# nmonette/TO-UED

Measured on NVIDIA B200. Metric: gridworld agent env-steps/sec incl. LPG update, higher is better.
Workload: dtype f16/bf16 operands, f32 accumulate (GRU); f32 elsewhere

## Files before the change

include/toued.h:

```cpp
#ifndef TOUED_H
#define TOUED_H
#include <stdint.h>
#ifdef __cplusplus
extern "C" {
#endif

#define TOUED_LEVEL_BYTES 192

const char* toued_last_error(void);
int toued_version(void);

int toued_rollout(const void* levels, const uint32_t* keys, const float* actor,
                  const uint8_t* forced_actions, int32_t* state, int32_t* obs, uint8_t* action,
                  float* reward, uint8_t* done, float* ep_return, int n_agents, int n_workers,
                  int rollout_len, int obs_dim, int max_grid_size, int max_n_objs, int reset_first,
                  void* stream);

int toued_env_step(const void* levels, const uint32_t* keys, const int32_t* actions, int32_t* state,
                   int32_t* obs, float* reward, uint8_t* done, int n_agents, int n_workers,
                   int max_grid_size, int max_n_objs, void* stream);
int toued_env_reset(const void* levels, int32_t* state, int32_t* obs, int n_agents, int n_workers,
                    int max_grid_size, void* stream);


int toued_sort_tokens(const int32_t* obs, uint16_t* sorted_tok, int n_agents, int n_workers,
                      int rollout_len, void* stream);

int toued_lpg_prepare(const int32_t* obs, const uint8_t* action, const float* reward,
                      const uint8_t* done, const float* actor, const float* critic,
                      const float* lpg_params, const int32_t* step, const void* levels, float* x,
                      void* ximg, int n_agents, int n_workers, int rollout_len, int obs_dim,
                      int lifetime_conditioning, int lpg_stride, void* stream);

int toued_gru_forward(const float* x, const uint8_t* done, const float* lpg_params, float* h_out,
                      float* gates, float* pi_hat, float* y_hat, int n_agents, int n_workers,
                      int rollout_len, int lifetime_conditioning, int lpg_stride, void* stream);

int toued_agent_scratch_floats(int n_agents, int n_workers, int rollout_len, int obs_dim);
int toued_agent_update(const int32_t* obs, const uint8_t* action, const uint16_t* sorted_tok,
                       const float* pi_hat, const float* y_hat, const float* actor_in,
                       const float* critic_in, float* actor_out, float* critic_out,
                       const void* levels, int32_t* step, float* scalars, int n_agents,
                       int n_workers, int rollout_len, int obs_dim, float lr_actor, float lr_critic,
                       float max_grad_norm, float agent_target_coeff, int tables_precopied, float* run_scratch,
                       void* stream);


int toued_meta_loss(const int32_t* obs, const uint8_t* action, const float* reward,
                    const uint8_t* done, const uint16_t* sorted_tok, const float* value_table,
                    const float* actor, float* lam, float* mu, float* scalars, int n_agents,
                    int n_workers, int rollout_len, int obs_dim, int value_stride, float gamma,
                    float gae_lambda, float grad_scale, int outer_product_quirk, void* stream);

int toued_agent_backward(const int32_t* obs, const uint8_t* action, const uint16_t* sorted_tok,
                         const float* pi_hat, const float* y_hat, const float* actor_k,
                         const float* critic_k, const float* actor_k1, const float* critic_k1,
                         const float* update_scalars, float* lam, float* mu, float* d_pi_hat,
                         float* d_y_hat, int n_agents, int n_workers, int rollout_len, int obs_dim,
                         float lr_actor, float lr_critic, float max_grad_norm,
                         float agent_target_coeff, float policy_entropy_coeff,
                         float target_entropy_coeff, float policy_l2_coeff, float target_l2_coeff,
                         float grad_scale, float* run_scratch, void* stream);

int toued_transpose_wh(const float* lpg_params, float* whT, void* stream);

int toued_gru_backward(const uint8_t* done, const float* lpg_params, const float* whT,
                       const float* h, float* gates, const float* y_hat, const float* d_pi_hat,
                       const float* d_y_hat, float* dl, float* dx, int n_agents, int n_workers,
                       int rollout_len, int lifetime_conditioning, void* stream);

int toued_lpg_wgrad_workspace_floats(void);
int toued_lpg_wgrad(const int32_t* obs, const uint8_t* done, const float* critic,
                    const float* lpg_params, const float* x, const float* h, const float* dgates,
                    const float* d_pi_hat, const float* dl, const float* dx, float* workspace,
                    int n_agents, int n_workers, int rollout_len, int obs_dim,
                    int lifetime_conditioning, int accumulate, void* stream);
int toued_lpg_wgrad_workspace_offset(int which);
int toued_lpg_wgrad_embed(const int32_t* obs, const uint8_t* done, const float* critic, const float* lpg_params,
                          const float* dx, float* workspace, const uint32_t* cotangent_max, int n_agents, int n_workers,
                          int rollout_len, int obs_dim, int lifetime_conditioning, int accumulate, void* stream);
int toued_lpg_wgrad_splits(int which);
int toued_reduce_partials(const float* workspace, float* grad, int lifetime_conditioning, int wh_splits,
                          int sm_splits, void* stream);

int toued_adam(float* params, const float* grad, float* mu, float* nu, int n, int count, float lr,
               float b1, float b2, float eps, void* stream);
int toued_adam_dev(float* params, const float* grad, float* mu, float* nu, int* count_dev, int n, float lr,
                   float b1, float b2, float eps, void* stream);
int toued_sgd_clip(float* params, const float* grad, float* sqnorm_scratch, int n, float lr, float max_norm,
                   void* stream);

int toued_a2c_update(const int32_t* obs, const uint8_t* action, const float* reward, const uint8_t* done,
                     const uint16_t* sorted_tok, const float* actor_in, const float* critic_in,
                     float* actor_out, float* critic_out, const void* levels, int32_t* step,
                     float* scalars, int n_agents, int n_workers, int rollout_len, int obs_dim,
                     float lr_actor, float lr_critic, float max_grad_norm, float gamma, float gae_lambda,
                     float entropy_coeff, int outer_product_quirk, void* stream);

int toued_a2c_train(const void* levels, const uint32_t* keys, float* actor0, float* actor1, float* critic0,
                    float* critic1, int32_t* state, int32_t* obs, uint8_t* action, float* reward, uint8_t* done,
                    uint16_t* sorted_tok, int32_t* step, float* scalars, float* loss_sums, int num_updates,
                    int n_agents, int n_workers, int rollout_len, int obs_dim, int max_grid_size, int max_n_objs,
                    float lr_actor, float lr_critic, float max_grad_norm, float gamma, float gae_lambda,
                    float entropy_coeff, int outer_product_quirk, void* stream);

int toued_es_ask(const uint32_t* key, const float* mean, float sigma, float* candidates, int popsize,
                 int n_params, int cand_stride, void* stream);
int toued_es_tell(const float* candidates, const float* fitness, float* mean, float* m, float* v,
                  int popsize, int n_params, int cand_stride, float sigma, float lrate, float beta1,
                  float beta2, float eps, int gen_counter, float mean_decay, void* stream);

int toued_es_ask_shard(const uint32_t* key, const float* mean, float sigma, float* candidates, int popsize_global,
                       int n_params, int cand_stride, int pair_offset, int n_pairs, void* stream);
int toued_es_grad_partial(const float* candidates, const float* fitness, const float* mean, float* grad_sum,
                          int n_members, int n_params, int cand_stride, float sigma, void* stream);
int toued_es_adam(const float* grad_sum, float* mean, float* m, float* v, int popsize_global, int n_params,
                  float sigma, float lrate, float beta1, float beta2, float eps, int gen_counter, float mean_decay,
                  void* stream);

int toued_plr_reset_lowest(float* score, uint8_t* active, uint8_t* is_new, int buffer_size, int minimum_new,
                           int* reset_ids, void* stream);
int toued_plr_select(uint32_t key0, uint32_t key1, float* score, uint8_t* active, uint8_t* is_new, int buffer_size,
                     const int* old_ids, const uint8_t* terminated, const float* new_scores, int n_agents,
                     float p_replay, float temperature, int shuffle_rounds, int* new_ids, void* stream);

int toued_generate_levels_desc_bytes(void);
int toued_generate_levels(const void* gen_desc, const uint32_t* keys, const int32_t* buffer_ids, void* levels_out,
                          int32_t* lifetimes_out, int n_levels, void* stream);

int toued_get_nash(const float* game, const float* x0, const float* y0, float* x_out, float* y_out,
                   int n, int x_nz, int y_nz, int num_iters, float lr, void* stream);
int toued_projection_simplex(float* v, int n, int max_nz, void* stream);


int toued_init_tables(const uint32_t* keys, const uint8_t* mask, float* tables, int n_agents,
                      int obs_dim, int n_out, void* stream);
int toued_masked_reset(const void* levels, const uint8_t* mask, int32_t* state, int32_t* obs,
                       int32_t* step, int n_agents, int n_workers, int max_grid_size, void* stream);

int toued_host_iota_bits(const uint32_t* keys, int n_keys, int n, uint32_t* out);


int toued_key_split(const uint32_t* keys_in, int n_keys, int num, int offset, int count, uint32_t* out,
                    void* stream);
int toued_key_chain(const uint32_t* keys_in, int n_keys, int chain_len, uint32_t* keys_out,
                    uint32_t* carry_out, void* stream);


int toued_tc_gemm_test(const float* A, const float* B, void* scratch_img, float* D, void* stream);
int toued_tc_gemm_mixed_test(const float* A, const float* B, void* scratch_img, float* D, void* stream);
int toued_tc_gemm_mn_test(const float* A, const float* B, void* scratch_img, float* D, int lbo, int sbo,
                          int kadv, void* stream);
int toued_tc_gemm_mn2_test(const float* A, const float* B, void* scratch_img, float* D, void* stream);

int toued_pack_wh_forward(const float* lpg_params, void* wh_img, int lifetime_conditioning, void* stream);
int toued_gru_forward_tc(const float* x, const uint8_t* done, const float* lpg_params, const void* wh_img,
                         void* h16, void* fac, void* hpimg, float* pi_hat, float* y_hat, int n_agents,
                         int n_workers, int rollout_len, int lifetime_conditioning, void* stream);
int toued_pack_wh_forward_multi(const float* lpg_params, void* wh_img, int lifetime_conditioning, int n_sets,
                                int lpg_stride, void* stream);
int toued_gru_forward_tc_multi(const float* x, const uint8_t* done, const float* lpg_params, const void* wh_img,
                               float* pi_hat, float* y_hat, int n_agents, int n_workers, int rollout_len,
                               int lifetime_conditioning, int lpg_stride, void* stream);

int toued_pack_wh_backward(const float* lpg_params, void* whb_img, void* stream);
int toued_cotangent_max(const float* d_pi_hat, const float* d_y_hat, int n_agents, int n_workers, int rollout_len,
                        uint32_t* cotangent_max, void* stream);
int toued_gru_backward_tc(const uint8_t* done, const float* lpg_params, const void* whb_img,
                          const void* h16, const void* fac, const float* y_hat, const float* d_pi_hat,
                          const float* d_y_hat, void* dgimg, float* dl, float* dx, const uint32_t* cotangent_max,
                          int n_agents, int n_workers, int rollout_len, int lifetime_conditioning, void* stream);
int toued_wgrad_tc_splits(void);
int toued_wgrad_tc_small_splits(void);
int toued_lpg_wgrad_tc(const void* hpimg, const void* dgimg, const void* ximg, const void* h16,
                       const float* d_pi_hat, const float* dl, float* wh_partials, float* small_partials,
                       const uint32_t* cotangent_max, int n_agents, int n_workers, int rollout_len, int accumulate,
                       void* stream);

#ifdef __cplusplus
}
#endif
#endif
```

to_ued_b200/_lib.py:

```python
from __future__ import annotations

import ctypes as C
import os

_HERE = os.path.dirname(os.path.abspath(__file__))
_VARIANT = os.environ.get("TOUED_LIB_VARIANT", "")
LIB_PATH = os.path.join(_HERE, f"libtoued_{_VARIANT}.so" if _VARIANT else "libtoued.so")

_lib = None


class TouedError(RuntimeError):
    pass


def lib() -> C.CDLL:
    global _lib
    if _lib is None:
        if not os.path.exists(LIB_PATH):
            raise TouedError(
                f"{LIB_PATH} is missing: the CUDA extension is not built. "
                "Run `python -m to_ued_b200.csrc.build` (there is no CPU fallback).")
        _lib = C.CDLL(LIB_PATH)
        _declare(_lib)
    return _lib


_P, _I, _F = C.c_void_p, C.c_int, C.c_float

SIGNATURES = {
    "toued_rollout": [_P] * 10 + [_I] * 7 + [_P],
    "toued_env_step": [_P] * 7 + [_I] * 4 + [_P],
    "toued_env_reset": [_P] * 3 + [_I] * 3 + [_P],
    "toued_sort_tokens": [_P] * 2 + [_I] * 3 + [_P],
    "toued_lpg_prepare": [_P] * 11 + [_I] * 6 + [_P],
    "toued_gru_forward": [_P] * 7 + [_I] * 5 + [_P],
    "toued_agent_update": [_P] * 12 + [_I] * 4 + [_F] * 4 + [_I, _P, _P],
    "toued_agent_scratch_floats": [_I] * 4,
    "toued_meta_loss": [_P] * 10 + [_I] * 5 + [_F] * 3 + [_I, _P],
    "toued_agent_backward": [_P] * 14 + [_I] * 4 + [_F] * 9 + [_P, _P],
    "toued_transpose_wh": [_P] * 3,
    "toued_gru_backward": [_P] * 10 + [_I] * 4 + [_P],
    "toued_lpg_wgrad_workspace_floats": [],
    "toued_lpg_wgrad": [_P] * 11 + [_I] * 6 + [_P],
    "toued_reduce_partials": [_P, _P, _I, _I, _I, _P],
    "toued_lpg_wgrad_splits": [_I],
    "toued_lpg_wgrad_workspace_offset": [_I],
    "toued_lpg_wgrad_embed": [_P] * 7 + [_I] * 6 + [_P],
    "toued_cotangent_max": [_P, _P, _I, _I, _I, _P, _P],
    "toued_pack_wh_backward": [_P] * 3,
    "toued_gru_backward_tc": [_P] * 12 + [_I] * 4 + [_P],
    "toued_wgrad_tc_splits": [],
    "toued_wgrad_tc_small_splits": [],
    "toued_lpg_wgrad_tc": [_P] * 9 + [_I] * 4 + [_P],
    "toued_adam": [_P] * 4 + [_I, _I] + [_F] * 4 + [_P],
    "toued_adam_dev": [_P] * 5 + [_I] + [_F] * 4 + [_P],
    "toued_sgd_clip": [_P] * 3 + [_I, _F, _F, _P],
    "toued_get_nash": [_P] * 5 + [_I] * 4 + [_F, _P],
    "toued_projection_simplex": [_P, _I, _I, _P],
    "toued_es_ask": [_P, _P, _F, _P, _I, _I, _I, _P],
    "toued_es_tell": [_P] * 5 + [_I, _I, _I] + [_F] * 5 + [_I, _F, _P],
    "toued_es_ask_shard": [_P, _P, _F, _P, _I, _I, _I, _I, _I, _P],
    "toued_es_grad_partial": [_P] * 4 + [_I, _I, _I, _F, _P],
    "toued_es_adam": [_P] * 4 + [_I, _I] + [_F] * 5 + [_I, _F, _P],
    "toued_a2c_update": [_P] * 12 + [_I] * 4 + [_F] * 6 + [_I, _P],
    "toued_a2c_train": [_P] * 15 + [_I] * 7 + [_F] * 6 + [_I, _P],
    "toued_init_tables": [_P] * 3 + [_I] * 3 + [_P],
    "toued_masked_reset": [_P] * 5 + [_I] * 3 + [_P],
    "toued_generate_levels_desc_bytes": [],
    "toued_generate_levels": [_P] * 5 + [_I, _P],
    "toued_plr_reset_lowest": [_P] * 3 + [_I, _I, _P, _P],
    "toued_plr_select": [C.c_uint32, C.c_uint32] + [_P] * 3 + [_I] + [_P] * 3 + [_I, _F, _F, _I, _P, _P],
    "toued_tc_gemm_test": [_P] * 5,
    "toued_tc_gemm_mixed_test": [_P] * 5,
    "toued_tc_gemm_mn_test": [_P] * 4 + [_I] * 3 + [_P],
    "toued_tc_gemm_mn2_test": [_P] * 5,
    "toued_pack_wh_forward": [_P, _P, _I, _P],
    "toued_pack_wh_forward_multi": [_P, _P, _I, _I, _I, _P],
    "toued_gru_forward_tc_multi": [_P] * 6 + [_I] * 5 + [_P],
    "toued_host_iota_bits": [_P, _I, _I, _P],
    "toued_key_split": [_P, _I, _I, _I, _I, _P, _P],
    "toued_key_chain": [_P, _I, _I, _P, _P, _P],
    "toued_gru_forward_tc": [_P] * 9 + [_I] * 4 + [_P],
}


def _declare(l):
    l.toued_last_error.restype = C.c_char_p
    l.toued_last_error.argtypes = []
    l.toued_version.restype = _I
    l.toued_version.argtypes = []
    for name, args in SIGNATURES.items():
        fn = getattr(l, name)
        fn.restype = _I
        fn.argtypes = args


def ptr(t):
    if t is None:
        return None
    if not t.is_cuda:
        raise TouedError("to_ued_b200 ops need CUDA tensors (there is no CPU fallback)")
    if not t.is_contiguous():
        raise TouedError("to_ued_b200 ops need contiguous tensors")
    return t.data_ptr()


def stream_ptr():
    import torch
    return torch.cuda.current_stream().cuda_stream


KERNELS_PER_CALL = {"toued_adam_dev": 2, "toued_sgd_clip": 2, "toued_lpg_wgrad": 3, "toued_init_tables": 2, "toued_lpg_wgrad_tc": 2, "toued_pack_wh_forward": 2, "toued_pack_wh_forward_multi": 2}
LAUNCHES = {}
GRAPH_KERNELS = [0]
ENV_STEPS = [0]
PROFILE = None


H2D_BYTES = [0]


def h2d(t):
    H2D_BYTES[0] += int(t.numel() * t.element_size()) if hasattr(t, "element_size") else int(t.nbytes)
    return t


def reset_counters(profile=False):
    global PROFILE
    H2D_BYTES[0] = 0
    GRAPH_KERNELS[0] = 0
    ENV_STEPS[0] = 0
    LAUNCHES.clear()
    PROFILE = {} if profile else None


def kernel_launches():
    return sum(n * KERNELS_PER_CALL.get(k, 1) for k, n in LAUNCHES.items()) + GRAPH_KERNELS[0]


def profile_ms():
    return {k: (len(v), sum(a.elapsed_time(b) for a, b in v)) for k, v in (PROFILE or {}).items()}


def call(name, *args):
    LAUNCHES[name] = LAUNCHES.get(name, 0) + 1
    if name == "toued_rollout":
        ENV_STEPS[0] += args[10] * args[11] * args[12]
    elif name == "toued_a2c_train":
        ENV_STEPS[0] += args[15] * args[16] * args[17] * args[18]
    if PROFILE is not None:
        import torch
        a, b = torch.cuda.Event(enable_timing=True), torch.cuda.Event(enable_timing=True)
        a.record()
        rc = getattr(lib(), name)(*args)
        b.record()
        PROFILE.setdefault(name, []).append((a, b))
    else:
        rc = getattr(lib(), name)(*args)
    if rc != 0:
        raise TouedError(f"{name} failed ({rc}): {lib().toued_last_error().decode()}")
```

to_ued_b200/agents/lpg_agent.py:

```python
from __future__ import annotations

from dataclasses import dataclass, field
from typing import Any, List, Optional

import numpy as np
import torch

from .. import _lib
from ..util import prng
from ..util.data import AgentState, Transition


@dataclass
class LPGAgentMetrics:
    policy_l2: Any
    policy_entropy: Any
    critic_loss: Any
    critic_l2: Any
    critic_entropy: Any

    def as_dict(self):
        return {"policy_l2": self.policy_l2, "policy_entropy": self.policy_entropy,
                "critic_loss": self.critic_loss, "critic_l2": self.critic_l2,
                "critic_entropy": self.critic_entropy}


class Tape:

    def __init__(self, n_agents, n_workers, rollout_len, obs_dim, num_updates, device, keep_gates=True,
                 precision=None, per_agent_params=False):
        import to_ued_b200
        N, W, L, D, K = n_agents, n_workers, rollout_len, obs_dim, num_updates
        R, dev = N * W, device
        f32, u8, i32 = torch.float32, torch.uint8, torch.int32
        self.N, self.W, self.L, self.D, self.K, self.R = N, W, L, D, K, R
        self.record = bool(keep_gates)
        kt = K + 1 if self.record else 2
        kr = K + 1 if self.record else 1
        ka = K if self.record else 1
        self.kt, self.kr, self.ka = kt, kr, ka
        self.actor = torch.empty((kt, N, D, 8), dtype=f32, device=dev)
        self.critic = torch.empty((kt, N, D, 8), dtype=f32, device=dev)
        self.obs = torch.empty((kr, N, L + 1, W), dtype=i32, device=dev)
        self.action = torch.empty((kr, N, L, W), dtype=u8, device=dev)
        self.reward = torch.empty((kr, N, L, W), dtype=f32, device=dev)
        self.done = torch.empty((kr, N, L, W), dtype=u8, device=dev)
        self.sorted_tok = torch.empty((kr, N, L * W), dtype=torch.int16, device=dev)
        self.precision = precision or to_ued_b200.GRU_PRECISION
        self.x = torch.empty((ka, L, R, 8), dtype=f32, device=dev)
        self.ximg = None
        if self.precision == "tc":
            f16 = torch.float16
            Rp = (R + 63) // 64 * 64
            R32 = (R + 31) // 32 * 32
            self.h16 = None if per_agent_params else torch.empty((ka, L, R32, 256), dtype=f16, device=dev)
            self.fac = torch.empty((ka, 4, L, R32, 256), dtype=f16, device=dev) if self.record else None
            self.hpimg = torch.zeros((ka, L * Rp * 256 * 2), dtype=torch.uint8, device=dev) if self.record else None
            self.ximg = torch.zeros((ka, L * Rp * 128), dtype=torch.uint8, device=dev) if self.record else None
            self.wh_img = torch.zeros((N if per_agent_params else 1) * 16 * 26624 // 2, dtype=f16, device=dev)
            self.h = self.gates = None
        else:
            self.h = torch.empty((ka, L, R, 256), dtype=f32, device=dev)
            self.gates = torch.empty((ka, 4, L, R, 256), dtype=f32, device=dev) if self.record else None
        self.pi_hat = torch.empty((ka, L, R), dtype=f32, device=dev)
        self.y_hat = torch.empty((ka, L, R, 8), dtype=f32, device=dev)
        self.scalars = torch.empty((ka, N, 8), dtype=f32, device=dev)
        self.scal_sum = torch.zeros((N, 8), dtype=f32, device=dev)
        self.step_in = torch.empty((ka, N), dtype=i32, device=dev)
        self.ep_return = torch.empty((N, W), dtype=f32, device=dev)
        self.agent_scratch = torch.empty(_lib.lib().toued_agent_scratch_floats(N, W, L, D), dtype=f32, device=dev)

    def ti(self, k):
        return k if self.record else (k & 1)

    def ri(self, k):
        return k if self.record else 0

    def ai(self, k):
        return k if self.record else 0

    def transition(self, k) -> Transition:
        r = self.ri(k)
        return Transition(self.obs[r], self.action[r], self.reward[r], self.done[r])


_SORT_STREAMS = {}


def _sort_stream(cur):
    key = (cur.device.index, cur.cuda_stream)
    st = _SORT_STREAMS.get(key)
    if st is None:
        st = _SORT_STREAMS[key] = torch.cuda.Stream(device=cur.device)
    return st


def _mark(label):
    import to_ued_b200
    if to_ued_b200.PHASE_EVENTS is not None and getattr(to_ued_b200, "PHASE_FINE", False):
        e = torch.cuda.Event(enable_timing=True)
        e.record(torch.cuda.current_stream())
        to_ued_b200.PHASE_EVENTS.append((label, -2, e))


def lpg_agent_train_step(k, tape: Tape, levels, step, lpg_params, lifetime_conditioning, agent_target_coeff,
                         lr_actor, lr_critic, max_grad_norm, lpg_stride=0):
    N, W, L, D = tape.N, tape.W, tape.L, tape.D
    s = _lib.stream_ptr()
    p = _lib.ptr
    r, a, t0, t1 = tape.ri(k), tape.ai(k), tape.ti(k), tape.ti(k + 1)
    import to_ued_b200
    cur = torch.cuda.current_stream()
    side = _sort_stream(cur) if to_ued_b200.SIDE_STREAMS else cur
    ev_roll, ev_sort = torch.cuda.Event(), torch.cuda.Event()
    ev_roll.record(cur)
    with torch.cuda.stream(side):
        side.wait_event(ev_roll)
        _lib.call("toued_sort_tokens", p(tape.obs[r]), p(tape.sorted_tok[r]), N, W, L, _lib.stream_ptr())
        precopied = bool(to_ued_b200.SIDE_STREAMS)
        if precopied:
            tape.actor[t1].copy_(tape.actor[t0])
            tape.critic[t1].copy_(tape.critic[t0])
        ev_sort.record(side)
    _mark("rollout")
    tape.step_in[a].copy_(step)
    _lib.call("toued_lpg_prepare", p(tape.obs[r]), p(tape.action[r]), p(tape.reward[r]), p(tape.done[r]),
              p(tape.actor[t0]), p(tape.critic[t0]), p(lpg_params), p(step), p(levels), p(tape.x[a]),
              p(tape.ximg[a]) if tape.ximg is not None else None,
              N, W, L, D, int(lifetime_conditioning), int(lpg_stride), s)
    if lpg_stride and tape.precision == "tc":
        _lib.call("toued_gru_forward_tc_multi", p(tape.x[a]), p(tape.done[r]), p(lpg_params), p(tape.wh_img),
                  p(tape.pi_hat[a]), p(tape.y_hat[a]), N, W, L, int(lifetime_conditioning), int(lpg_stride), s)
    elif lpg_stride or tape.precision != "tc":
        _lib.call("toued_gru_forward", p(tape.x[a]), p(tape.done[r]), p(lpg_params), p(tape.h[a]),
                  p(tape.gates[a]) if tape.gates is not None else None, p(tape.pi_hat[a]), p(tape.y_hat[a]),
                  N, W, L, int(lifetime_conditioning), int(lpg_stride), s)
    else:
        _lib.call("toued_gru_forward_tc", p(tape.x[a]), p(tape.done[r]), p(lpg_params), p(tape.wh_img),
                  p(tape.h16[a]), p(tape.fac[a]) if tape.fac is not None else None,
                  p(tape.hpimg[a]) if tape.hpimg is not None else None, p(tape.pi_hat[a]), p(tape.y_hat[a]),
                  N, W, L, int(lifetime_conditioning), s)
    _mark("gru_fwd")
    cur.wait_event(ev_sort)
    _mark("sort_wait")
    _lib.call("toued_agent_update", p(tape.obs[r]), p(tape.action[r]), p(tape.sorted_tok[r]), p(tape.pi_hat[a]),
              p(tape.y_hat[a]), p(tape.actor[t0]), p(tape.critic[t0]), p(tape.actor[t1]), p(tape.critic[t1]),
              p(levels), p(step), p(tape.scalars[a]), N, W, L, D, float(lr_actor), float(lr_critic),
              float(max_grad_norm), float(agent_target_coeff), int(precopied), p(tape.agent_scratch), s)
    tape.scal_sum += tape.scalars[a]
    _mark("update")


def train_lpg_agent_steps(rng, lpg_train_state, agent_state: AgentState, rollout_manager, num_train_steps: int,
                          agent_target_coeff: float, tape: Optional[Tape] = None, lpg_stride: int = 0):
    env = rollout_manager.env
    actor, critic = agent_state.actor_state, agent_state.critic_state
    N, W = agent_state.env_state.packed.shape
    L, K = rollout_manager.train_rollout_len, num_train_steps
    dev = actor.params.device
    if tape is None:
        import to_ued_b200
        tape = Tape(N, W, L, env.obs_dim, K, dev, keep_gates=False,
                    precision=to_ued_b200.ES_PRECISION if lpg_stride else None, per_agent_params=bool(lpg_stride))
    levels = agent_state.level.packed
    step = actor.step.clone()
    state = agent_state.env_state.packed.clone()
    tape.actor[0].copy_(actor.params)
    tape.critic[0].copy_(critic.params)
    tape.scal_sum.zero_()
    keys_d = prng.chain_device(prng.to_device(rng, dev), K)
    p = _lib.ptr
    lpg = lpg_train_state.params if hasattr(lpg_train_state, "params") else lpg_train_state
    cond = lpg_train_state.model.lifetime_conditioning if hasattr(lpg_train_state, "model") else False
    if tape.precision == "tc" and not lpg_stride:
        _lib.call("toued_pack_wh_forward", p(lpg), p(tape.wh_img), int(cond), _lib.stream_ptr())
    elif tape.precision == "tc":
        _lib.call("toued_pack_wh_forward_multi", p(lpg), p(tape.wh_img), int(cond), N, int(lpg_stride), _lib.stream_ptr())
    yield
    for k in range(K):
        r = tape.ri(k)
        _lib.call("toued_rollout", p(levels), p(keys_d[k]), p(tape.actor[tape.ti(k)]), None, p(state), p(tape.obs[r]),
                  p(tape.action[r]), p(tape.reward[r]), p(tape.done[r]), None, N, W, L, env.obs_dim,
                  env.max_grid_size, env.max_n_objs, 0, _lib.stream_ptr())
        lpg_agent_train_step(k, tape, levels, step, lpg, cond, agent_target_coeff, actor.learning_rate,
                             critic.learning_rate, actor.max_grad_norm, lpg_stride=lpg_stride)
        yield
    sc = tape.scal_sum / K
    metrics = LPGAgentMetrics(policy_l2=sc[:, 4], policy_entropy=sc[:, 6], critic_loss=sc[:, 3],
                              critic_l2=sc[:, 5], critic_entropy=sc[:, 7])
    from ..environments.gridworld.gridworld import EnvState
    new_agent = agent_state.replace(
        actor_state=actor.replace(params=tape.actor[tape.ti(K)].clone(), step=step),
        critic_state=critic.replace(params=tape.critic[tape.ti(K)].clone(), step=step.clone()),
        env_obs=tape.obs[tape.ri(K - 1)][:, -1].clone(), env_state=EnvState(state, env.max_n_objs))
    rollouts = [tape.transition(k) for k in range(K)] if tape.record else [tape.transition(K - 1)]
    return new_agent, rollouts, metrics


def train_lpg_agent(rng, lpg_train_state, agent_state: AgentState, rollout_manager, num_train_steps: int,
                    agent_target_coeff: float, tape: Optional[Tape] = None, lpg_stride: int = 0):
    gen = train_lpg_agent_steps(rng, lpg_train_state, agent_state, rollout_manager, num_train_steps,
                                agent_target_coeff, tape=tape, lpg_stride=lpg_stride)
    while True:
        try:
            next(gen)
        except StopIteration as done:
            return done.value
```

to_ued_b200/csrc/agent_backward.cu:

```cuda
#include "lpg_common.cuh"
#include "segreduce.cuh"
#include "../../include/toued.h"

__global__ void __launch_bounds__(256)
meta_loss_kernel(const int32_t* __restrict__ obs, const uint8_t* __restrict__ action,
                 const float* __restrict__ reward, const uint8_t* __restrict__ done,
                 const uint16_t* __restrict__ sorted_tok, const float* __restrict__ value,
                 const float* __restrict__ actor, float* __restrict__ lam, float* __restrict__ mu,
                 float* __restrict__ scal, int W, int L, int D, int vstride, float gamma, float lmbda,
                 float gscale, int quirk) {
    extern __shared__ __align__(16) float sm[];
    float* adv = sm;
    float* rec = adv + L * W;
    float* abar = rec + L * W * 6;
    float* lbar = abar + W;
    float* runv = lbar + W;
    float* scan = runv + L * W * 5;
    void* idxmem = scan + 2 * 256 * 5;
    __shared__ float red[32];
    __shared__ int iscan[512];
    __shared__ unsigned char sflags[512];
    const int n = blockIdx.x, tid = threadIdx.x, T = W * L;
    const int32_t* ob = obs + (size_t)n * (L + 1) * W;
    const uint8_t* act = action + (size_t)n * T;
    const float* rw = reward + (size_t)n * T;
    const uint8_t* dn = done + (size_t)n * T;
    const uint16_t* st = sorted_tok + (size_t)n * T;
    const float* vt = value + (size_t)n * D * vstride;
    const float* at = actor + (size_t)n * D * 8;
    float* lm = lam + (size_t)n * D * 8;
    float* mm = mu + (size_t)n * D * 8;
    const float invT = 1.0f / (float)T;
    const SegIndex si = seg_index_build(idxmem, iscan, st, ob, T);

    for (int i = tid; i < D * 2; i += 256) {
        reinterpret_cast<float4*>(lm)[i] = make_float4(0.f, 0.f, 0.f, 0.f);
        reinterpret_cast<float4*>(mm)[i] = make_float4(0.f, 0.f, 0.f, 0.f);
    }
    float s1 = 0.f, s2 = 0.f;
    const float vlast = vt[(size_t)(D - 1) * vstride];
    for (int w = tid; w < W; w += 256) {
        float g = 0.f;
        int32_t o1 = ob[L * W + w];
        float v1 = vt[(size_t)ob_idx(o1) * vstride] + 0.001f * (float)ob_time(o1) * vlast;
        for (int t = L - 1; t >= 0; --t) {
            const int32_t o0 = ob[t * W + w];
            const float v0 = vt[(size_t)ob_idx(o0) * vstride] + 0.001f * (float)ob_time(o0) * vlast;
            const float nd = dn[t * W + w] ? 0.0f : 1.0f;
            const float delta = rw[t * W + w] + gamma * v1 * nd - v0;
            g = delta + gamma * lmbda * nd * g;
            adv[t * W + w] = g;
            s1 += g; s2 = fmaf(g, g, s2);
            v1 = v0;
        }
    }
    s1 = block_sum(s1, red); s2 = block_sum(s2, red);
    const float mean = s1 * invT;
    float var = 0.f;
    for (int i = tid; i < T; i += 256) { const float d = adv[i] - mean; var = fmaf(d, d, var); }
    var = block_sum(var, red) * invT;
    const float inv_std = 1.0f / (sqrtf(var) + 1e-8f);
    __syncthreads();
    for (int i = tid; i < T; i += 256) adv[i] = (adv[i] - mean) * inv_std;
    __syncthreads();
    for (int tok = tid; tok < T; tok += 256) {
        const int32_t o = ob[tok];
        float z[5], p[5];
        tab_logits8<5>(at, D, o, z);
        softmax_c<5>(z, p);
        const int a = act[tok];
        float pa = p[0];
#pragma unroll
        for (int j = 1; j < 5; ++j) pa = (a == j) ? p[j] : pa;
        float* r = rec + tok * 6;
        r[5] = logf(pa + 1e-8f);
        const float q = pa / (pa + 1e-8f);
#pragma unroll
        for (int j = 0; j < 5; ++j) r[j] = q * ((a == j ? 1.0f : 0.0f) - p[j]);
    }
    __syncthreads();
    float loss = 0.f;
    for (int w = tid; w < W; w += 256) {
        float sa = 0.f, sl = 0.f, se = 0.f;
        for (int t = 0; t < L; ++t) { sa += adv[t * W + w]; sl += rec[(t * W + w) * 6 + 5]; se = fmaf(adv[t * W + w], rec[(t * W + w) * 6 + 5], se); }
        abar[w] = sa / (float)L; lbar[w] = sl / (float)L;
        loss -= quirk ? abar[w] * lbar[w] : se / (float)L;
    }
    loss = block_sum(loss, red) / (float)W;
    __syncthreads();
    float last[5] = {0.f, 0.f, 0.f, 0.f, 0.f};
    for (int tok = tid; tok < T; tok += 256) {
        const int w = tok % W;
        const float coef = -gscale * invT * (quirk ? abar[w] : adv[tok]);
        float* r = rec + tok * 6;
        const float tf = 0.001f * (float)ob_time(ob[tok]);
#pragma unroll
        for (int j = 0; j < 5; ++j) { r[j] *= coef; last[j] = fmaf(tf, r[j], last[j]); }
        r[5] = tf;
    }
#pragma unroll
    for (int j = 0; j < 5; ++j) last[j] = block_sum(last[j], red);
    __syncthreads();
    seg_reduce<5, 6>(rec, si, T, runv, scan, sflags);
    for (int r = tid; r < si.nruns; r += 256) {
        const int row = si.run_row[r];
#pragma unroll
        for (int j = 0; j < 5; ++j) lm[(size_t)row * 8 + j] = runv[r * 5 + j];
    }
    if (tid == 0) {
#pragma unroll
        for (int j = 0; j < 5; ++j) lm[(size_t)(D - 1) * 8 + j] = last[j];
        scal[n * 2 + 0] = loss;
        scal[n * 2 + 1] = s2 * invT;
    }
}

extern "C" int toued_meta_loss(const int32_t* obs, const uint8_t* action, const float* reward,
                               const uint8_t* done, const uint16_t* sorted_tok, const float* value_table,
                               const float* actor, float* lam, float* mu, float* scalars, int n_agents,
                               int n_workers, int rollout_len, int obs_dim, int value_stride, float gamma,
                               float gae_lambda, float grad_scale, int outer_product_quirk, void* stream) {
    const int T = n_workers * rollout_len;
    TOUED_CHECK(n_agents > 0 && T > 0, "toued_meta_loss: empty problem");
    const size_t smem = sizeof(float) * ((size_t)T * 7 + 2 * n_workers + (size_t)T * 5 + 2 * 256 * 5) + seg_index_bytes(T);
    TOUED_CHECK(smem <= 200 * 1024, "toued_meta_loss: W*L=%d too large for shared memory", T);
    TOUED_CUDA(cudaFuncSetAttribute(meta_loss_kernel, cudaFuncAttributeMaxDynamicSharedMemorySize, (int)smem));
    meta_loss_kernel<<<n_agents, 256, smem, (cudaStream_t)stream>>>(
        obs, action, reward, done, sorted_tok, value_table, actor, lam, mu, scalars, n_workers, rollout_len,
        obs_dim, value_stride, gamma, gae_lambda, grad_scale, outer_product_quirk);
    TOUED_LAUNCH_CHECK();
    return 0;
}

struct TokFwd { float p[5], y[8], pa, q, tf; int a; };

__device__ __forceinline__ TokFwd tok_forward(const float* at, const float* ct, int D, int32_t o, int a) {
    TokFwd f;
    float z[5], zy[8];
    tab_logits8<5>(at, D, o, z);
    softmax_c<5>(z, f.p);
    tab_logits8<8>(ct, D, o, zy);
    softmax_c<8>(zy, f.y);
    f.a = a;
    f.pa = f.p[0];
#pragma unroll
    for (int j = 1; j < 5; ++j) f.pa = (a == j) ? f.p[j] : f.pa;
    f.q = f.pa / (f.pa + 1e-8f);
    f.tf = 0.001f * (float)ob_time(o);
    return f;
}

__device__ __forceinline__ void tok_grad(const TokFwd& f, float ph, const float* yh, float invT, float alpha, float* c) {
    const float ca = invT * ph * f.q;
#pragma unroll
    for (int j = 0; j < 5; ++j) c[j] = ca * ((f.a == j ? 1.0f : 0.0f) - f.p[j]);
    float mm[8], b = 0.f;
#pragma unroll
    for (int i = 0; i < 8; ++i) {
        mm[i] = logf(f.y[i] + 1e-8f) - logf(yh[i] + 1e-8f) + f.y[i] / (f.y[i] + 1e-8f);
        b = fmaf(f.y[i], mm[i], b);
    }
    const float cc = alpha * invT;
#pragma unroll
    for (int i = 0; i < 8; ++i) c[5 + i] = cc * f.y[i] * (mm[i] - b);
}

__device__ __forceinline__ void load8(const float* p, float* v) {
    const float4 a = reinterpret_cast<const float4*>(p)[0], b = reinterpret_cast<const float4*>(p)[1];
    v[0] = a.x; v[1] = a.y; v[2] = a.z; v[3] = a.w; v[4] = b.x; v[5] = b.y; v[6] = b.z; v[7] = b.w;
}

__global__ void __launch_bounds__(256, 2)
agent_backward_kernel(const int32_t* __restrict__ obs, const uint8_t* __restrict__ action,
                      const uint16_t* __restrict__ sorted_tok, const float* __restrict__ pi_hat,
                      const float* __restrict__ y_hat, const float* __restrict__ actor_k,
                      const float* __restrict__ critic_k, const float* __restrict__ actor_k1,
                      const float* __restrict__ critic_k1, const float* __restrict__ upd_scal,
                      float* lam, float* mu, float* __restrict__ d_pi_hat, float* __restrict__ d_y_hat,
                      float* run_scratch, int n_agents, int W, int L, int D, float lr_a, float lr_c, float max_norm,
                      float alpha, float b_pent, float b_yent, float b_pl2, float b_yl2, float gscale) {
    extern __shared__ __align__(16) float rec[];
    __shared__ float red[32];
    __shared__ float s_wlast[13];
    __shared__ int iscan[512];
    __shared__ unsigned char sflags[512];
    const int n = blockIdx.x, tid = threadIdx.x, T = W * L, R = n_agents * W;
    const int32_t* ob = obs + (size_t)n * (L + 1) * W;
    const uint8_t* act = action + (size_t)n * T;
    const uint16_t* st = sorted_tok + (size_t)n * T;
    const float* a0 = actor_k + (size_t)n * D * 8;
    const float* c0 = critic_k + (size_t)n * D * 8;
    const float* a1 = actor_k1 + (size_t)n * D * 8;
    const float* c1 = critic_k1 + (size_t)n * D * 8;
    float* lm = lam + (size_t)n * D * 8;
    float* mm = mu + (size_t)n * D * 8;
    const float invT = 1.0f / (float)T;
    const float gna = upd_scal[n * 8 + 0], gnc = upd_scal[n * 8 + 1];
    const bool keep = upd_scal[n * 8 + 2] != 0.0f;
    float* runv = run_scratch + (size_t)n * min(T, D) * 13;
    float* scan = rec + (size_t)T * 13;
    const SegIndex si = seg_index_build(scan + 2 * 256 * 13, iscan, st, ob, T);

    float last[13];
#pragma unroll
    for (int j = 0; j < 13; ++j) last[j] = 0.f;
    for (int tok = tid; tok < T; tok += 256) {
        const TokFwd f = tok_forward(a1, c1, D, ob[tok], act[tok]);
        float* r = rec + tok * 13;
        {
            float dh[5], s = 0.f;
#pragma unroll
            for (int j = 0; j < 5; ++j) { dh[j] = -(logf(f.p[j] + 1e-8f) + 1.0f); s = fmaf(f.p[j], dh[j], s); }
            const float k = -b_pent * gscale * invT;
#pragma unroll
            for (int j = 0; j < 5; ++j) r[j] = k * f.p[j] * (dh[j] - s);
        }
        {
            float dh[8], s = 0.f;
#pragma unroll
            for (int j = 0; j < 8; ++j) { dh[j] = -(logf(f.y[j] + 1e-8f) + 1.0f); s = fmaf(f.y[j], dh[j], s); }
            const float k = -b_yent * gscale * invT;
#pragma unroll
            for (int j = 0; j < 8; ++j) r[5 + j] = k * f.y[j] * (dh[j] - s);
        }
#pragma unroll
        for (int j = 0; j < 13; ++j) last[j] = fmaf(f.tf, r[j], last[j]);
    }
#pragma unroll
    for (int j = 0; j < 13; ++j) last[j] = block_sum(last[j], red);
    __syncthreads();
    seg_reduce<13, 13>(rec, si, T, runv, scan, sflags);
    for (int r = tid; r < si.nruns; r += 256) {
        const int row = si.run_row[r];
        const float* g = runv + r * 13;
#pragma unroll
        for (int j = 0; j < 5; ++j) lm[(size_t)row * 8 + j] += g[j];
#pragma unroll
        for (int j = 0; j < 8; ++j) mm[(size_t)row * 8 + j] += g[5 + j];
    }
    if (tid == 0) {
#pragma unroll
        for (int j = 0; j < 5; ++j) lm[(size_t)(D - 1) * 8 + j] += last[j];
#pragma unroll
        for (int j = 0; j < 8; ++j) mm[(size_t)(D - 1) * 8 + j] += last[5 + j];
    }
    __syncthreads();

    const float dir_pi = gscale * b_pl2 * 2.0f * invT;
    const float dir_y = gscale * b_yl2 * 2.0f * invT;
    if (!keep) {
        for (int tok = tid; tok < T; tok += 256) {
            const int t = tok / W, w = tok - t * W;
            const size_t li = (size_t)t * R + (size_t)n * W + w;
            d_pi_hat[li] = dir_pi * pi_hat[li];
            float yh[8]; load8(y_hat + li * 8, yh);
            float4* o = reinterpret_cast<float4*>(d_y_hat + li * 8);
            o[0] = make_float4(dir_y * yh[0], dir_y * yh[1], dir_y * yh[2], dir_y * yh[3]);
            o[1] = make_float4(dir_y * yh[4], dir_y * yh[5], dir_y * yh[6], dir_y * yh[7]);
        }
        return;
    }

#pragma unroll
    for (int j = 0; j < 13; ++j) last[j] = 0.f;
    for (int tok = tid; tok < T; tok += 256) {
        const int t = tok / W, w = tok - t * W;
        const size_t li = (size_t)t * R + (size_t)n * W + w;
        const TokFwd f = tok_forward(a0, c0, D, ob[tok], act[tok]);
        float yh[8]; load8(y_hat + li * 8, yh);
        float* r = rec + tok * 13;
        tok_grad(f, pi_hat[li], yh, invT, alpha, r);
#pragma unroll
        for (int j = 0; j < 13; ++j) last[j] = fmaf(f.tf, r[j], last[j]);
    }
#pragma unroll
    for (int j = 0; j < 13; ++j) last[j] = block_sum(last[j], red);
    __syncthreads();
    seg_reduce<13, 13>(rec, si, T, runv, scan, sflags);
    float dot_a = 0.f, dot_c = 0.f;
    for (int r = tid; r < si.nruns; r += 256) {
        const int row = si.run_row[r];
        const float* g = runv + r * 13;
        float l8[8], m8[8];
        load8(lm + (size_t)row * 8, l8); load8(mm + (size_t)row * 8, m8);
#pragma unroll
        for (int j = 0; j < 5; ++j) dot_a = fmaf(g[j], l8[j], dot_a);
#pragma unroll
        for (int j = 0; j < 8; ++j) dot_c = fmaf(g[5 + j], m8[j], dot_c);
    }
    dot_a = block_sum(dot_a, red); dot_c = block_sum(dot_c, red);
    float ll[8], ml[8];
    load8(lm + (size_t)(D - 1) * 8, ll); load8(mm + (size_t)(D - 1) * 8, ml);
#pragma unroll
    for (int j = 0; j < 5; ++j) dot_a = fmaf(last[j], ll[j], dot_a);
#pragma unroll
    for (int j = 0; j < 8; ++j) dot_c = fmaf(last[5 + j], ml[j], dot_c);
    const bool clip_a = !(gna < max_norm), clip_c = !(gnc < max_norm);
    const float ka = -lr_a * (clip_a ? max_norm / gna : 1.0f), pa_ = clip_a ? dot_a / (gna * gna) : 0.0f;
    const float kc = -lr_c * (clip_c ? max_norm / gnc : 1.0f), pc_ = clip_c ? dot_c / (gnc * gnc) : 0.0f;
    if (tid == 0) {
#pragma unroll
        for (int j = 0; j < 5; ++j) s_wlast[j] = ka * (ll[j] - pa_ * last[j]);
#pragma unroll
        for (int j = 0; j < 8; ++j) s_wlast[5 + j] = kc * (ml[j] - pc_ * last[5 + j]);
    }
    __syncthreads();
    float wl[13];
#pragma unroll
    for (int j = 0; j < 13; ++j) wl[j] = s_wlast[j];

    for (int r = tid; r < si.nruns; r += 256) {
        const int row = si.run_row[r];
        float* g = runv + r * 13;
        float l8[8], m8[8];
        load8(lm + (size_t)row * 8, l8); load8(mm + (size_t)row * 8, m8);
#pragma unroll
        for (int j = 0; j < 5; ++j) g[j] = ka * (l8[j] - pa_ * g[j]);
#pragma unroll
        for (int j = 0; j < 8; ++j) g[5 + j] = kc * (m8[j] - pc_ * g[5 + j]);
    }
    __syncthreads();
    float hl[13];
#pragma unroll
    for (int j = 0; j < 13; ++j) hl[j] = 0.f;
    for (int pos = tid; pos < T; pos += 256) {
        const int tok = si.tok[pos];
        const int t = tok / W, w = tok - t * W;
        const size_t li = (size_t)t * R + (size_t)n * W + w;
        const TokFwd f = tok_forward(a0, c0, D, ob[tok], act[tok]);
        const float ph = pi_hat[li];
        float yh[8]; load8(y_hat + li * 8, yh);
        float* r = rec + tok * 13;
        const float* wr = runv + (size_t)si.run[pos] * 13;
        float v[13];
#pragma unroll
        for (int j = 0; j < 13; ++j) v[j] = fmaf(f.tf, wl[j], wr[j]);
        float va = v[0], pv = 0.f;
#pragma unroll
        for (int j = 1; j < 5; ++j) va = (f.a == j) ? v[j] : va;
#pragma unroll
        for (int j = 0; j < 5; ++j) pv = fmaf(f.p[j], v[j], pv);
        const float s = va - pv;
        d_pi_hat[li] = invT * f.q * s + dir_pi * ph;
        const float pe = f.pa + 1e-8f;
        const float c1_ = ph * invT * s * 1e-8f * f.pa / (pe * pe), c2_ = ph * invT * f.q;
        float h[13];
#pragma unroll
        for (int j = 0; j < 5; ++j)
            h[j] = c1_ * ((f.a == j ? 1.0f : 0.0f) - f.p[j]) - c2_ * f.p[j] * (v[j] - pv);
        float m[8], mp[8], av = 0.f, b = 0.f;
#pragma unroll
        for (int j = 0; j < 8; ++j) {
            const float ye = f.y[j] + 1e-8f;
            m[j] = logf(ye) - logf(yh[j] + 1e-8f) + f.y[j] / ye;
            mp[j] = (f.y[j] + 2e-8f) / (ye * ye);
            av = fmaf(v[5 + j], f.y[j], av);
            b = fmaf(f.y[j], m[j], b);
        }
        const float ca = alpha * invT;
        float dS[8], sy = 0.f, dyo[8];
#pragma unroll
        for (int j = 0; j < 8; ++j) {
            const float vc = v[5 + j];
            dyo[j] = ca * f.y[j] * (av - vc) / (yh[j] + 1e-8f) + dir_y * yh[j];
            dS[j] = vc * m[j] + vc * f.y[j] * mp[j] - vc * b - av * (m[j] + f.y[j] * mp[j]);
            sy = fmaf(f.y[j], dS[j], sy);
        }
#pragma unroll
        for (int j = 0; j < 8; ++j) h[5 + j] = ca * f.y[j] * (dS[j] - sy);
        float4* o = reinterpret_cast<float4*>(d_y_hat + li * 8);
        o[0] = make_float4(dyo[0], dyo[1], dyo[2], dyo[3]);
        o[1] = make_float4(dyo[4], dyo[5], dyo[6], dyo[7]);
#pragma unroll
        for (int j = 0; j < 13; ++j) { r[j] = h[j]; hl[j] = fmaf(f.tf, h[j], hl[j]); }
    }
#pragma unroll
    for (int j = 0; j < 13; ++j) hl[j] = block_sum(hl[j], red);
    __syncthreads();
    seg_reduce<13, 13>(rec, si, T, runv, scan, sflags);
    for (int r = tid; r < si.nruns; r += 256) {
        const int row = si.run_row[r];
        const float* g = runv + r * 13;
#pragma unroll
        for (int j = 0; j < 5; ++j) lm[(size_t)row * 8 + j] += g[j];
#pragma unroll
        for (int j = 0; j < 8; ++j) mm[(size_t)row * 8 + j] += g[5 + j];
    }
    if (tid == 0) {
#pragma unroll
        for (int j = 0; j < 5; ++j) lm[(size_t)(D - 1) * 8 + j] = ll[j] + hl[j];
#pragma unroll
        for (int j = 0; j < 8; ++j) mm[(size_t)(D - 1) * 8 + j] = ml[j] + hl[5 + j];
    }
}

extern "C" int toued_agent_backward(const int32_t* obs, const uint8_t* action, const uint16_t* sorted_tok,
                                    const float* pi_hat, const float* y_hat, const float* actor_k,
                                    const float* critic_k, const float* actor_k1, const float* critic_k1,
                                    const float* update_scalars, float* lam, float* mu, float* d_pi_hat,
                                    float* d_y_hat, int n_agents, int n_workers, int rollout_len, int obs_dim,
                                    float lr_actor, float lr_critic, float max_grad_norm,
                                    float agent_target_coeff, float policy_entropy_coeff,
                                    float target_entropy_coeff, float policy_l2_coeff, float target_l2_coeff,
                                    float grad_scale, float* run_scratch, void* stream) {
    const int T = n_workers * rollout_len;
    TOUED_CHECK(n_agents > 0 && T > 0, "toued_agent_backward: empty problem");
    TOUED_CHECK(run_scratch != nullptr, "toued_agent_backward: run_scratch (toued_agent_scratch_floats) is required");
    const size_t smem = sizeof(float) * ((size_t)T * 13 + 2 * 256 * 13) + seg_index_bytes(T);
    TOUED_CHECK(smem <= 200 * 1024, "toued_agent_backward: W*L=%d too large for shared memory", T);
    TOUED_CUDA(cudaFuncSetAttribute(agent_backward_kernel, cudaFuncAttributeMaxDynamicSharedMemorySize, (int)smem));
    TOUED_CUDA(cudaFuncSetAttribute(agent_backward_kernel, cudaFuncAttributePreferredSharedMemoryCarveout, 100));
    cudaStream_t st = (cudaStream_t)stream;
    agent_backward_kernel<<<n_agents, 256, smem, st>>>(
        obs, action, sorted_tok, pi_hat, y_hat, actor_k, critic_k, actor_k1, critic_k1, update_scalars, lam, mu,
        d_pi_hat, d_y_hat, run_scratch, n_agents, n_workers, rollout_len, obs_dim, lr_actor, lr_critic, max_grad_norm,
        agent_target_coeff, policy_entropy_coeff, target_entropy_coeff, policy_l2_coeff, target_l2_coeff, grad_scale);
    TOUED_LAUNCH_CHECK();
    return 0;
}
```

to_ued_b200/csrc/agent_update.cu:

```cuda
#include "lpg_common.cuh"
#include "segreduce.cuh"
#include "../../include/toued.h"

constexpr int AU_C = 13;

__global__ void __launch_bounds__(256, 2)
agent_update_kernel(const int32_t* __restrict__ obs, const uint8_t* __restrict__ action,
                    const uint16_t* __restrict__ sorted_tok, const float* __restrict__ pi_hat,
                    const float* __restrict__ y_hat, const float* __restrict__ actor_in,
                    const float* __restrict__ critic_in, float* actor_out, float* critic_out,
                    const LevelRec* __restrict__ levels, int32_t* __restrict__ step,
                    float* __restrict__ scal, float* run_scratch, int n_agents, int W, int L, int D,
                    float lr_a, float lr_c, float max_norm, float alpha, int tables_precopied) {
    extern __shared__ __align__(16) float smc[];
    __shared__ float red[32];
    __shared__ int iscan[512];
    __shared__ unsigned char sflags[512];
    const int n = blockIdx.x, tid = threadIdx.x, T = W * L, R = n_agents * W;
    float* runv = run_scratch + (size_t)n * min(T, D) * 13;
    float* scan = smc + (size_t)T * AU_C;
    void* idxmem = scan + 2 * 256 * 13;
    const int32_t* ob = obs + (size_t)n * (L + 1) * W;
    const uint8_t* act = action + (size_t)n * T;
    const float* a_in = actor_in + (size_t)n * D * 8;
    const float* c_in = critic_in + (size_t)n * D * 8;
    float* a_out = actor_out + (size_t)n * D * 8;
    float* c_out = critic_out + (size_t)n * D * 8;
    const float invT = 1.0f / (float)T;
    const SegIndex si = seg_index_build(idxmem, iscan, sorted_tok + (size_t)n * T, ob, T);

    if (!tables_precopied)
        for (int i = tid; i < D * 2; i += 256) {
            reinterpret_cast<float4*>(a_out)[i] = reinterpret_cast<const float4*>(a_in)[i];
            reinterpret_cast<float4*>(c_out)[i] = reinterpret_cast<const float4*>(c_in)[i];
        }

    float m_kl = 0.f, m_pi2 = 0.f, m_y2 = 0.f;
    float last[13];
#pragma unroll
    for (int j = 0; j < 13; ++j) last[j] = 0.f;
    for (int tok = tid; tok < T; tok += 256) {
        const int t = tok / W, w = tok - t * W;
        const size_t li = (size_t)t * R + (size_t)n * W + w;
        const int32_t o = ob[tok];
        float z[5], p[5], zy[8], y[8];
        tab_logits8<5>(a_in, D, o, z);
        softmax_c<5>(z, p);
        tab_logits8<8>(c_in, D, o, zy);
        softmax_c<8>(zy, y);
        const int a = act[tok];
        float pa = p[0];
#pragma unroll
        for (int j = 1; j < 5; ++j) pa = (a == j) ? p[j] : pa;
        const float ph = pi_hat[li];
        const float ca = invT * ph * (pa / (pa + 1e-8f));
        float* rec = smc + tok * AU_C;
#pragma unroll
        for (int j = 0; j < 5; ++j) rec[j] = ca * ((a == j ? 1.0f : 0.0f) - p[j]);
        float yh[8];
        { const float4* q = reinterpret_cast<const float4*>(y_hat + li * 8); const float4 q0 = q[0], q1 = q[1];
          yh[0] = q0.x; yh[1] = q0.y; yh[2] = q0.z; yh[3] = q0.w; yh[4] = q1.x; yh[5] = q1.y; yh[6] = q1.z; yh[7] = q1.w; }
        float mm[8], b = 0.f, kl = 0.f, y2 = 0.f;
#pragma unroll
        for (int i = 0; i < 8; ++i) {
            const float ly = logf(y[i] + 1e-8f), lh = logf(yh[i] + 1e-8f);
            mm[i] = ly - lh + y[i] / (y[i] + 1e-8f);
            b = fmaf(y[i], mm[i], b);
            kl = fmaf(y[i], ly - lh, kl);
            y2 = fmaf(yh[i], yh[i], y2);
        }
        const float cc = alpha * invT;
#pragma unroll
        for (int i = 0; i < 8; ++i) rec[5 + i] = cc * y[i] * (mm[i] - b);
        const float tf = 0.001f * (float)ob_time(o);
#pragma unroll
        for (int j = 0; j < 13; ++j) last[j] = fmaf(tf, rec[j], last[j]);
        m_kl += kl; m_pi2 = fmaf(ph, ph, m_pi2); m_y2 += y2;
    }
#pragma unroll
    for (int j = 0; j < 13; ++j) last[j] = block_sum(last[j], red);
    m_kl = block_sum(m_kl, red); m_pi2 = block_sum(m_pi2, red); m_y2 = block_sum(m_y2, red);
    __syncthreads();

    seg_reduce<13, AU_C>(smc, si, T, runv, scan, sflags);
    float na = 0.f, nc = 0.f;
    for (int r = tid; r < si.nruns; r += 256) {
        const float* g = runv + r * 13;
#pragma unroll
        for (int j = 0; j < 5; ++j) na = fmaf(g[j], g[j], na);
#pragma unroll
        for (int j = 5; j < 13; ++j) nc = fmaf(g[j], g[j], nc);
    }
    na = block_sum(na, red); nc = block_sum(nc, red);
#pragma unroll
    for (int j = 0; j < 5; ++j) na = fmaf(last[j], last[j], na);
#pragma unroll
    for (int j = 5; j < 13; ++j) nc = fmaf(last[j], last[j], nc);
    const float gna = sqrtf(na), gnc = sqrtf(nc);
    const float sa = gna < max_norm ? 1.0f : max_norm / gna;
    const float sc = gnc < max_norm ? 1.0f : max_norm / gnc;
    const int old_step = step[n];
    const bool keep = (old_step + 1) <= levels[n].lifetime;
    const float ua = keep ? lr_a * sa : 0.0f, uc = keep ? lr_c * sc : 0.0f;

    for (int r = tid; r < si.nruns; r += 256) {
        const int row = si.run_row[r];
        const float* g = runv + r * 13;
#pragma unroll
        for (int j = 0; j < 5; ++j) a_out[(size_t)row * 8 + j] = a_in[(size_t)row * 8 + j] - ua * g[j];
#pragma unroll
        for (int j = 0; j < 8; ++j) c_out[(size_t)row * 8 + j] = c_in[(size_t)row * 8 + j] - uc * g[5 + j];
    }
    if (tid == 0) {
#pragma unroll
        for (int j = 0; j < 5; ++j) a_out[(size_t)(D - 1) * 8 + j] = a_in[(size_t)(D - 1) * 8 + j] - ua * last[j];
#pragma unroll
        for (int j = 0; j < 8; ++j) c_out[(size_t)(D - 1) * 8 + j] = c_in[(size_t)(D - 1) * 8 + j] - uc * last[5 + j];
        step[n] = keep ? old_step + 1 : old_step;
    }
    __syncthreads();

    float ea = 0.f, ec = 0.f;
    for (int tok = tid; tok < T; tok += 256) {
        const int32_t o = ob[tok];
        float z[5], p[5], zy[8], y[8];
        tab_logits8<5>(a_out, D, o, z);
        softmax_c<5>(z, p);
        tab_logits8<8>(c_out, D, o, zy);
        softmax_c<8>(zy, y);
#pragma unroll
        for (int j = 0; j < 5; ++j) { const float q = p[j] + 1e-8f; ea -= q * logf(q); }
#pragma unroll
        for (int j = 0; j < 8; ++j) { const float q = y[j] + 1e-8f; ec -= q * logf(q); }
    }
    ea = block_sum(ea, red); ec = block_sum(ec, red);
    if (tid == 0) {
        float* s = scal + (size_t)n * 8;
        s[0] = gna; s[1] = gnc; s[2] = keep ? 1.0f : 0.0f;
        s[3] = m_kl * invT;
        s[4] = m_pi2 * invT;
        s[5] = m_y2 * invT;
        s[6] = ea * invT;
        s[7] = ec * invT;
    }
}

static size_t agent_smem_bytes(int T, int D) {
    return sizeof(float) * ((size_t)T * AU_C + 2 * 256 * 13) + seg_index_bytes(T);
}

extern "C" int toued_agent_update(const int32_t* obs, const uint8_t* action, const uint16_t* sorted_tok,
                                  const float* pi_hat, const float* y_hat, const float* actor_in,
                                  const float* critic_in, float* actor_out, float* critic_out,
                                  const void* levels, int32_t* step, float* scalars, int n_agents,
                                  int n_workers, int rollout_len, int obs_dim, float lr_actor,
                                  float lr_critic, float max_grad_norm, float agent_target_coeff, int tables_precopied,
                                  float* run_scratch, void* stream) {
    const int T = n_workers * rollout_len;
    const size_t smem = agent_smem_bytes(T, obs_dim);
    TOUED_CHECK(n_agents > 0 && T > 0, "toued_agent_update: empty problem");
    TOUED_CHECK(smem <= 200 * 1024, "toued_agent_update: W*L=%d too large for shared memory", T);
    TOUED_CHECK(actor_in != actor_out && critic_in != critic_out, "toued_agent_update: in-place update not supported");
    TOUED_CUDA(cudaFuncSetAttribute(agent_update_kernel, cudaFuncAttributeMaxDynamicSharedMemorySize, (int)smem));
    TOUED_CUDA(cudaFuncSetAttribute(agent_update_kernel, cudaFuncAttributePreferredSharedMemoryCarveout, 100));
    TOUED_CHECK(run_scratch != nullptr, "toued_agent_update: run_scratch (toued_agent_scratch_floats) is required");
    cudaStream_t st = (cudaStream_t)stream;
    agent_update_kernel<<<n_agents, 256, smem, st>>>(
        obs, action, sorted_tok, pi_hat, y_hat, actor_in, critic_in, actor_out, critic_out,
        (const LevelRec*)levels, step, scalars, run_scratch, n_agents, n_workers, rollout_len, obs_dim,
        lr_actor, lr_critic, max_grad_norm, agent_target_coeff, tables_precopied);
    TOUED_LAUNCH_CHECK();
    return 0;
}

extern "C" int toued_agent_scratch_floats(int n_agents, int n_workers, int rollout_len, int obs_dim) {
    const long long T = (long long)n_workers * rollout_len;
    const long long n = 13ll * (T < obs_dim ? T : obs_dim) * n_agents;
    return n < (1ll << 31) ? (int)n : -1;
}
```

to_ued_b200/csrc/lpg_backward.cu:

```cuda
#include "lpg_common.cuh"
#include "tc.cuh"
#include "../../include/toued.h"

__device__ __forceinline__ void cp_async16z(void* smem, const void* gmem, bool valid) {
    const int sz = valid ? 16 : 0;
    asm volatile("cp.async.cg.shared.global [%0], [%1], 16, %2;" ::"r"(smem_u32(smem)), "l"(gmem), "r"(sz));
}
__device__ __forceinline__ void cp_commit() { asm volatile("cp.async.commit_group;"); }
template <int N> __device__ __forceinline__ void cp_wait() { asm volatile("cp.async.wait_group %0;" ::"n"(N)); }

__global__ void transpose_wh_kernel(const float* __restrict__ Wh, float* __restrict__ WhT) {
    __shared__ float tile[32][33];
    const int c0 = blockIdx.x * 32, j0 = blockIdx.y * 32;
    for (int r = threadIdx.y; r < 32; r += 8) tile[r][threadIdx.x] = Wh[(size_t)(j0 + r) * LPG_G + c0 + threadIdx.x];
    __syncthreads();
    for (int r = threadIdx.y; r < 32; r += 8) WhT[(size_t)(c0 + r) * LPG_H + j0 + threadIdx.x] = tile[threadIdx.x][r];
}

constexpr int GB_TM = 64;
constexpr int GB_KC = 16;
constexpr int GB_CS = LPG_H + 4;
constexpr int GB_AS = GB_KC + 4;

__global__ void __launch_bounds__(256, 1)
gru_backward_kernel(const uint8_t* __restrict__ done, const float* __restrict__ lpg, int X,
                    const float* __restrict__ WhT, const float* __restrict__ h, float* gates,
                    const float* __restrict__ y_hat, const float* __restrict__ d_pi_hat,
                    const float* __restrict__ d_y_hat, float* __restrict__ dl_out,
                    float* __restrict__ dx, int R, int L, int W) {
    extern __shared__ __align__(16) float sm[];
    float* C = sm;
    float* As = C + GB_TM * GB_CS;
    float* Bs = As + 2 * GB_TM * GB_AS;
    float* swp = Bs + 2 * GB_KC * LPG_H;
    float* sWy = swp + LPG_H;
    float* sWi = sWy + LPG_H * LPG_Y;
    __shared__ float snd[GB_TM];
    const LpgOffsets o = lpg_offsets(X);
    const int tid = threadIdx.x;
    const int row0 = blockIdx.x * GB_TM;
    const int nrows = min(GB_TM, R - row0);
    const size_t gs = (size_t)L * R * LPG_H;

    for (int i = tid; i < LPG_H; i += 256) swp[i] = lpg[o.w_pi + i];
    for (int i = tid; i < LPG_H * LPG_Y; i += 256) sWy[i] = lpg[o.W_y + i];
    for (int i = tid; i < 2 * LPG_G; i += 256) sWi[i] = lpg[o.Wi + 3 * LPG_G + i];
    for (int i = tid; i < GB_TM * GB_CS; i += 256) C[i] = 0.0f;
    __syncthreads();

    const int rl = tid >> 2, part = tid & 3;
    const int rg = tid >> 5, cg = tid & 31;

    for (int t = 0; t < L; ++t) {
        if (tid < GB_TM) {
            const int r = row0 + tid;
            snd[tid] = (tid < nrows && !done[((size_t)(r / W) * L + t) * W + (r % W)]) ? 1.0f : 0.0f;
        }
        __syncthreads();
        float dx3 = 0.f, dx4 = 0.f;
        const size_t tok = (size_t)t * R + row0 + rl;
        if (rl < nrows) {
            float yh[8], dy[8], dl[8];
            { const float4* q = reinterpret_cast<const float4*>(y_hat + tok * 8); const float4 a = q[0], b = q[1];
              yh[0] = a.x; yh[1] = a.y; yh[2] = a.z; yh[3] = a.w; yh[4] = b.x; yh[5] = b.y; yh[6] = b.z; yh[7] = b.w; }
            { const float4* q = reinterpret_cast<const float4*>(d_y_hat + tok * 8); const float4 a = q[0], b = q[1];
              dy[0] = a.x; dy[1] = a.y; dy[2] = a.z; dy[3] = a.w; dy[4] = b.x; dy[5] = b.y; dy[6] = b.z; dy[7] = b.w; }
            float s = 0.f;
#pragma unroll
            for (int i = 0; i < 8; ++i) s = fmaf(yh[i], dy[i], s);
#pragma unroll
            for (int i = 0; i < 8; ++i) dl[i] = yh[i] * (dy[i] - s);
            const float dpi = d_pi_hat[tok];
            if (part == 0) {
                float4* q = reinterpret_cast<float4*>(dl_out + tok * 8);
                q[0] = make_float4(dl[0], dl[1], dl[2], dl[3]);
                q[1] = make_float4(dl[4], dl[5], dl[6], dl[7]);
            }
            const bool has_next = (t + 1 < L) && snd[rl] != 0.0f;
            const size_t base = tok * LPG_H + part * 64;
            for (int j4 = 0; j4 < 64; j4 += 4) {
                const int j = part * 64 + j4;
                const float4 rr = *reinterpret_cast<const float4*>(gates + base + j4);
                const float4 zz = *reinterpret_cast<const float4*>(gates + gs + base + j4);
                const float4 nn = *reinterpret_cast<const float4*>(gates + 2 * gs + base + j4);
                const float4 hn = *reinterpret_cast<const float4*>(gates + 3 * gs + base + j4);
                const float4 ht = *reinterpret_cast<const float4*>(h + base + j4);
                float4 hp = make_float4(0.f, 0.f, 0.f, 0.f);
                if (has_next) hp = *reinterpret_cast<const float4*>(h + base + j4 + (size_t)R * LPG_H);
                const float4 cr = *reinterpret_cast<const float4*>(C + rl * GB_CS + j);
                float r_[4] = {rr.x, rr.y, rr.z, rr.w}, z_[4] = {zz.x, zz.y, zz.z, zz.w};
                float n_[4] = {nn.x, nn.y, nn.z, nn.w}, hn_[4] = {hn.x, hn.y, hn.z, hn.w};
                float ht_[4] = {ht.x, ht.y, ht.z, ht.w}, hp_[4] = {hp.x, hp.y, hp.z, hp.w};
                float c_[4] = {cr.x, cr.y, cr.z, cr.w};
                float dar[4], daz[4], dan[4], dhn[4], cz[4];
#pragma unroll
                for (int e = 0; e < 4; ++e) {
                    const int u = j + e;
                    float dh = c_[e];
                    if (ht_[e] > 0.0f) {
                        float hd = dpi * swp[u];
#pragma unroll
                        for (int i = 0; i < 8; ++i) hd = fmaf(dl[i], sWy[u * 8 + i], hd);
                        dh += hd;
                    }
                    const float dn = dh * (1.0f - z_[e]);
                    const float dz = dh * (hp_[e] - n_[e]);
                    dan[e] = dn * (1.0f - n_[e] * n_[e]);
                    dhn[e] = dan[e] * r_[e];
                    dar[e] = dan[e] * hn_[e] * r_[e] * (1.0f - r_[e]);
                    daz[e] = dz * z_[e] * (1.0f - z_[e]);
                    cz[e] = dh * z_[e];
                    dx3 = fmaf(dar[e], sWi[u], fmaf(daz[e], sWi[LPG_H + u], fmaf(dan[e], sWi[2 * LPG_H + u], dx3)));
                    dx4 = fmaf(dar[e], sWi[LPG_G + u], fmaf(daz[e], sWi[LPG_G + LPG_H + u], fmaf(dan[e], sWi[LPG_G + 2 * LPG_H + u], dx4)));
                }
                *reinterpret_cast<float4*>(gates + base + j4) = make_float4(dar[0], dar[1], dar[2], dar[3]);
                *reinterpret_cast<float4*>(gates + gs + base + j4) = make_float4(daz[0], daz[1], daz[2], daz[3]);
                *reinterpret_cast<float4*>(gates + 2 * gs + base + j4) = make_float4(dan[0], dan[1], dan[2], dan[3]);
                *reinterpret_cast<float4*>(gates + 3 * gs + base + j4) = make_float4(dhn[0], dhn[1], dhn[2], dhn[3]);
                *reinterpret_cast<float4*>(C + rl * GB_CS + j) = make_float4(cz[0], cz[1], cz[2], cz[3]);
            }
        }
        dx3 += __shfl_xor_sync(0xffffffffu, dx3, 1); dx3 += __shfl_xor_sync(0xffffffffu, dx3, 2);
        dx4 += __shfl_xor_sync(0xffffffffu, dx4, 1); dx4 += __shfl_xor_sync(0xffffffffu, dx4, 2);
        if (part == 0 && rl < nrows) *reinterpret_cast<float2*>(dx + tok * 2) = make_float2(dx3, dx4);
        __syncthreads();
        if (t + 1 == L) break;
        float acc[8][8];
#pragma unroll
        for (int i = 0; i < 8; ++i)
#pragma unroll
            for (int j = 0; j < 8; ++j) acc[i][j] = 0.f;
        auto load_chunk = [&](int buf, int c0) {
            const int gate = c0 >> 8, u0 = c0 & 255;
            const size_t plane = (size_t)(gate == 2 ? 3 : gate) * gs;
            {
                const int r = tid >> 2, q = tid & 3;
                const bool ok = r < nrows;
                const float* src = gates + plane + ((size_t)t * R + row0 + (ok ? r : 0)) * LPG_H + u0 + q * 4;
                cp_async16z(As + (buf * GB_TM + r) * GB_AS + q * 4, src, ok);
            }
#pragma unroll
            for (int q = 0; q < 4; ++q) {
                const int f = tid + q * 256, kk = f >> 6, c4 = f & 63;
                cp_async16z(Bs + (buf * GB_KC + kk) * LPG_H + c4 * 4, WhT + (size_t)(c0 + kk) * LPG_H + c4 * 4, true);
            }
            cp_commit();
        };
        load_chunk(0, 0);
        for (int kc = 0; kc < LPG_G / GB_KC; ++kc) {
            if (kc + 1 < LPG_G / GB_KC) { load_chunk((kc + 1) & 1, (kc + 1) * GB_KC); cp_wait<1>(); }
            else cp_wait<0>();
            __syncthreads();
            const float* as = As + (kc & 1) * GB_TM * GB_AS;
            const float* bs = Bs + (kc & 1) * GB_KC * LPG_H;
#pragma unroll
            for (int k4 = 0; k4 < GB_KC; k4 += 4) {
                float4 a[8];
#pragma unroll
                for (int i = 0; i < 8; ++i) a[i] = *reinterpret_cast<const float4*>(as + (rg * 8 + i) * GB_AS + k4);
#pragma unroll
                for (int kk = 0; kk < 4; ++kk) {
                    const float4 b0 = *reinterpret_cast<const float4*>(bs + (k4 + kk) * LPG_H + cg * 4);
                    const float4 b1 = *reinterpret_cast<const float4*>(bs + (k4 + kk) * LPG_H + 128 + cg * 4);
#pragma unroll
                    for (int i = 0; i < 8; ++i) {
                        const float av = kk == 0 ? a[i].x : kk == 1 ? a[i].y : kk == 2 ? a[i].z : a[i].w;
                        acc[i][0] = fmaf(av, b0.x, acc[i][0]); acc[i][1] = fmaf(av, b0.y, acc[i][1]);
                        acc[i][2] = fmaf(av, b0.z, acc[i][2]); acc[i][3] = fmaf(av, b0.w, acc[i][3]);
                        acc[i][4] = fmaf(av, b1.x, acc[i][4]); acc[i][5] = fmaf(av, b1.y, acc[i][5]);
                        acc[i][6] = fmaf(av, b1.z, acc[i][6]); acc[i][7] = fmaf(av, b1.w, acc[i][7]);
                    }
                }
            }
            __syncthreads();
        }
#pragma unroll
        for (int i = 0; i < 8; ++i) {
            const int r = rg * 8 + i;
            const float nd = snd[r];
            float4* c0p = reinterpret_cast<float4*>(C + r * GB_CS + cg * 4);
            float4* c1p = reinterpret_cast<float4*>(C + r * GB_CS + 128 + cg * 4);
            const float4 c0 = *c0p, c1 = *c1p;
            *c0p = make_float4(nd * (acc[i][0] + c0.x), nd * (acc[i][1] + c0.y), nd * (acc[i][2] + c0.z), nd * (acc[i][3] + c0.w));
            *c1p = make_float4(nd * (acc[i][4] + c1.x), nd * (acc[i][5] + c1.y), nd * (acc[i][6] + c1.z), nd * (acc[i][7] + c1.w));
        }
        __syncthreads();
    }
}

static size_t gru_bwd_smem() {
    return sizeof(float) * (GB_TM * GB_CS + 2 * GB_TM * GB_AS + 2 * GB_KC * LPG_H + LPG_H + LPG_H * LPG_Y + 2 * LPG_G);
}

extern "C" int toued_gru_backward(const uint8_t* done, const float* lpg_params, const float* whT,
                                  const float* h, float* gates, const float* y_hat, const float* d_pi_hat,
                                  const float* d_y_hat, float* dl, float* dx, int n_agents, int n_workers,
                                  int rollout_len, int lifetime_conditioning, void* stream) {
    const int R = n_agents * n_workers;
    TOUED_CHECK(R > 0 && rollout_len > 0, "toued_gru_backward: empty problem");
    const size_t smem = gru_bwd_smem();
    TOUED_CUDA(cudaFuncSetAttribute(gru_backward_kernel, cudaFuncAttributeMaxDynamicSharedMemorySize, (int)smem));
    gru_backward_kernel<<<(R + GB_TM - 1) / GB_TM, 256, smem, (cudaStream_t)stream>>>(
        done, lpg_params, lifetime_conditioning ? 7 : 5, whT, h, gates, y_hat, d_pi_hat, d_y_hat, dl, dx, R,
        rollout_len, n_workers);
    TOUED_LAUNCH_CHECK();
    return 0;
}

extern "C" int toued_transpose_wh(const float* lpg_params, float* whT, void* stream) {
    transpose_wh_kernel<<<dim3(LPG_G / 32, LPG_H / 32), dim3(32, 8), 0, (cudaStream_t)stream>>>(
        lpg_params + lpg_offsets(5).Wh, whT);
    TOUED_LAUNCH_CHECK();
    return 0;
}

constexpr int WG_KC = 16;
__global__ void __launch_bounds__(256)
wgrad_wh_kernel(const uint8_t* __restrict__ done, const float* __restrict__ h, const float* __restrict__ gates,
                float* __restrict__ partial, int R, int L, int W, int chunks_per_split, int accumulate) {
    __shared__ __align__(16) float As[2][WG_KC][64];
    __shared__ __align__(16) float Bs[2][WG_KC][64];
    const int tid = threadIdx.x;
    const int c0 = blockIdx.x * 64, j0 = blockIdx.y * 64, split = blockIdx.z;
    const int gate = c0 >> 8, u0 = c0 & 255;
    const size_t gs = (size_t)L * R * LPG_H;
    const float* gp = gates + (size_t)(gate == 2 ? 3 : gate) * gs;
    const size_t ntok = (size_t)L * R;
    const size_t tok_begin = (size_t)split * chunks_per_split * WG_KC;
    const int tj = tid >> 4, tc = tid & 15;
    float acc[4][4];
#pragma unroll
    for (int i = 0; i < 4; ++i)
#pragma unroll
        for (int j = 0; j < 4; ++j) acc[i][j] = 0.f;
    auto load_chunk = [&](int buf, int ch) {
        const int kk = tid >> 4, q = tid & 15;
        const size_t tok = tok_begin + (size_t)ch * WG_KC + kk;
        const bool in = tok < ntok;
        const int t = in ? (int)(tok / R) : 0;
        const int row = in ? (int)(tok % R) : 0;
        const bool has_next = in && (t + 1 < L) && !done[((size_t)(row / W) * L + t) * W + (row % W)];
        const float* asrc = h + ((size_t)(has_next ? t + 1 : 0) * R + row) * LPG_H + j0 + q * 4;
        cp_async16z(&As[buf][kk][q * 4], asrc, has_next);
        const float* bsrc = gp + (in ? tok : 0) * LPG_H + u0 + q * 4;
        cp_async16z(&Bs[buf][kk][q * 4], bsrc, in);
        cp_commit();
    };
    load_chunk(0, 0);
    for (int ch = 0; ch < chunks_per_split; ++ch) {
        if (ch + 1 < chunks_per_split) { load_chunk((ch + 1) & 1, ch + 1); cp_wait<1>(); }
        else cp_wait<0>();
        __syncthreads();
        const int b = ch & 1;
#pragma unroll
        for (int kk = 0; kk < WG_KC; ++kk) {
            const float4 a = *reinterpret_cast<const float4*>(&As[b][kk][tj * 4]);
            const float4 v = *reinterpret_cast<const float4*>(&Bs[b][kk][tc * 4]);
            const float a_[4] = {a.x, a.y, a.z, a.w};
#pragma unroll
            for (int i = 0; i < 4; ++i) {
                acc[i][0] = fmaf(a_[i], v.x, acc[i][0]); acc[i][1] = fmaf(a_[i], v.y, acc[i][1]);
                acc[i][2] = fmaf(a_[i], v.z, acc[i][2]); acc[i][3] = fmaf(a_[i], v.w, acc[i][3]);
            }
        }
        __syncthreads();
    }
    float* out = partial + (size_t)split * LPG_H * LPG_G;
#pragma unroll
    for (int i = 0; i < 4; ++i) {
        float4* p = reinterpret_cast<float4*>(out + (size_t)(j0 + tj * 4 + i) * LPG_G + c0 + tc * 4);
        float4 v = make_float4(acc[i][0], acc[i][1], acc[i][2], acc[i][3]);
        if (accumulate) { const float4 pv = *p; v.x += pv.x; v.y += pv.y; v.z += pv.z; v.w += pv.w; }
        *p = v;
    }
}

constexpr int SM_WI = 0, SM_BHN = 8 * LPG_G, SM_WPI = SM_BHN + LPG_H, SM_WY = SM_WPI + LPG_H,
              SM_BPI = SM_WY + LPG_H * LPG_Y, SM_BY = SM_BPI + 1, SM_TOTAL = SM_BY + LPG_Y;

__global__ void __launch_bounds__(256)
wgrad_small_kernel(const float* __restrict__ x, const float* __restrict__ h, const float* __restrict__ gates,
                   const float* __restrict__ d_pi_hat, const float* __restrict__ dl, float* __restrict__ partial,
                   int R, int L, int toks_per_split, int accumulate) {
    const int j = threadIdx.x, split = blockIdx.x;
    const size_t ntok = (size_t)L * R, gs = ntok * LPG_H;
    const size_t t0 = (size_t)split * toks_per_split;
    const size_t t1 = min(ntok, t0 + (size_t)toks_per_split);
    float wi[3][8], bhn = 0.f, head[9], hb = 0.f;
#pragma unroll
    for (int g = 0; g < 3; ++g)
#pragma unroll
        for (int q = 0; q < 8; ++q) wi[g][q] = 0.f;
#pragma unroll
    for (int i = 0; i < 9; ++i) head[i] = 0.f;
    for (size_t tok = t0; tok < t1; ++tok) {
        const float4 x0 = *reinterpret_cast<const float4*>(x + tok * 8), x1 = *reinterpret_cast<const float4*>(x + tok * 8 + 4);
        const float xv[8] = {x0.x, x0.y, x0.z, x0.w, x1.x, x1.y, x1.z, x1.w};
        const float4 d0 = *reinterpret_cast<const float4*>(dl + tok * 8), d1 = *reinterpret_cast<const float4*>(dl + tok * 8 + 4);
        const float dv[9] = {d_pi_hat[tok], d0.x, d0.y, d0.z, d0.w, d1.x, d1.y, d1.z, d1.w};
        const float dar = gates[tok * LPG_H + j], daz = gates[gs + tok * LPG_H + j];
        const float dan = gates[2 * gs + tok * LPG_H + j], dhn = gates[3 * gs + tok * LPG_H + j];
        const float y = fmaxf(h[tok * LPG_H + j], 0.0f);
#pragma unroll
        for (int q = 0; q < 8; ++q) {
            wi[0][q] = fmaf(xv[q], dar, wi[0][q]); wi[1][q] = fmaf(xv[q], daz, wi[1][q]); wi[2][q] = fmaf(xv[q], dan, wi[2][q]);
        }
        bhn += dhn;
#pragma unroll
        for (int i = 0; i < 9; ++i) head[i] = fmaf(y, dv[i], head[i]);
        if (j < 9) hb += dv[j];
    }
    float* out = partial + (size_t)split * SM_TOTAL;
    auto put = [&](int idx, float v) { out[idx] = accumulate ? out[idx] + v : v; };
#pragma unroll
    for (int g = 0; g < 3; ++g)
#pragma unroll
        for (int q = 0; q < 8; ++q) put(SM_WI + q * LPG_G + g * LPG_H + j, wi[g][q]);
    put(SM_BHN + j, bhn);
    put(SM_WPI + j, head[0]);
#pragma unroll
    for (int i = 0; i < 8; ++i) put(SM_WY + j * 8 + i, head[1 + i]);
    if (j < 9) put(SM_BPI + j, hb);
}

constexpr int EM_TOTAL = LPG_Y * LPG_E + 2 * LPG_E + 1;
constexpr int EM_SREC = 44;
__global__ void __launch_bounds__(256, 2)
embed_backward_kernel(const int32_t* __restrict__ obs, const uint8_t* __restrict__ done,
                      const float* __restrict__ critic, const float* __restrict__ lpg, int emb_off,
                      const float* __restrict__ dx, float* __restrict__ partial, const uint32_t* __restrict__ cotmax,
                      int n_agents, int W, int L, int D, int accumulate) {
    __shared__ float sp[EM_TOTAL];
    __shared__ float part[4][EM_TOTAL + 3];
    const float inv_s = cotmax ? 1.0f / cot_scale_from_max(*cotmax) : 1.0f;
    extern __shared__ __align__(16) float srec[];
    const int tid = threadIdx.x;
    for (int i = tid; i < EM_TOTAL; i += 256) sp[i] = lpg[emb_off + i];
    __syncthreads();
    const size_t total = (size_t)n_agents * L * W;
    const size_t R = (size_t)n_agents * W;
    const size_t iters = (total + (size_t)gridDim.x * 256 - 1) / ((size_t)gridDim.x * 256);
    const int grp = tid >> 6, lt = tid & 63;
    int src = -1, ysrc = -1, out0 = 0, nout = 0;
    if (lt < 32)      { ysrc = lt >> 2; src = 8 + 4 * (lt & 3); out0 = (lt >> 2) * LPG_E + 4 * (lt & 3); nout = 4; }
    else if (lt < 36) { src = 8 + 4 * (lt - 32); out0 = LPG_Y * LPG_E + 4 * (lt - 32); nout = 4; }
    else if (lt < 40) { src = 8 + LPG_E + 4 * (lt - 36); out0 = LPG_Y * LPG_E + LPG_E + 4 * (lt - 36); nout = 4; }
    else if (lt == 40) { src = 8 + 2 * LPG_E; out0 = LPG_Y * LPG_E + 2 * LPG_E; nout = 1; }
    float acc[4] = {0.f, 0.f, 0.f, 0.f};
    for (size_t it = 0; it < iters; ++it) {
        const size_t g = (it * gridDim.x + blockIdx.x) * 256 + tid;
        const bool ok = g < total;
        float y[2][8], dp[2] = {0.f, 0.f};
#pragma unroll
        for (int s = 0; s < 2; ++s)
#pragma unroll
            for (int i = 0; i < 8; ++i) y[s][i] = 0.f;
        if (ok) {
            const int w = (int)(g % W), t = (int)((g / W) % L), n = (int)(g / ((size_t)W * L));
            const float* ct = critic + (size_t)n * D * 8;
            float zy[8];
            tab_logits8<8>(ct, D, obs[((size_t)n * (L + 1) + t) * W + w], zy);
            softmax_c<8>(zy, y[0]);
            tab_logits8<8>(ct, D, obs[((size_t)n * (L + 1) + t + 1) * W + w], zy);
            softmax_c<8>(zy, y[1]);
            const float2 d = *reinterpret_cast<const float2*>(dx + ((size_t)t * R + (size_t)n * W + w) * 2);
            dp[0] = d.x * inv_s;
            dp[1] = done[g] ? 0.0f : d.y * inv_s;
        }
        float* r0 = srec + (size_t)tid * EM_SREC;
        float* r1 = srec + (size_t)(256 + tid) * EM_SREC;
        reinterpret_cast<float4*>(r0)[0] = make_float4(y[0][0], y[0][1], y[0][2], y[0][3]);
        reinterpret_cast<float4*>(r0)[1] = make_float4(y[0][4], y[0][5], y[0][6], y[0][7]);
        reinterpret_cast<float4*>(r1)[0] = make_float4(y[1][0], y[1][1], y[1][2], y[1][3]);
        reinterpret_cast<float4*>(r1)[1] = make_float4(y[1][4], y[1][5], y[1][6], y[1][7]);
#pragma unroll
        for (int eq = 0; eq < LPG_E / 4; ++eq) {
            float da[2][4], rd[2][4];
#pragma unroll
            for (int k = 0; k < 4; ++k) {
                const int e = eq * 4 + k;
                float a0 = sp[LPG_Y * LPG_E + e], a1 = a0;
#pragma unroll
                for (int i = 0; i < 8; ++i) {
                    const float wgt = sp[i * LPG_E + e];
                    a0 = fmaf(y[0][i], wgt, a0);
                    a1 = fmaf(y[1][i], wgt, a1);
                }
                const float w1 = sp[LPG_Y * LPG_E + LPG_E + e];
                da[0][k] = a0 > 0.0f ? dp[0] * w1 : 0.0f;   rd[0][k] = fmaxf(a0, 0.0f) * dp[0];
                da[1][k] = a1 > 0.0f ? dp[1] * w1 : 0.0f;   rd[1][k] = fmaxf(a1, 0.0f) * dp[1];
            }
            reinterpret_cast<float4*>(r0 + 8)[eq] = make_float4(da[0][0], da[0][1], da[0][2], da[0][3]);
            reinterpret_cast<float4*>(r0 + 8 + LPG_E)[eq] = make_float4(rd[0][0], rd[0][1], rd[0][2], rd[0][3]);
            reinterpret_cast<float4*>(r1 + 8)[eq] = make_float4(da[1][0], da[1][1], da[1][2], da[1][3]);
            reinterpret_cast<float4*>(r1 + 8 + LPG_E)[eq] = make_float4(rd[1][0], rd[1][1], rd[1][2], rd[1][3]);
        }
        r0[8 + 2 * LPG_E] = dp[0];
        r1[8 + 2 * LPG_E] = dp[1];
        __syncthreads();
        if (nout == 4) {
            const float* base = srec + (size_t)grp * 128 * EM_SREC;
#pragma unroll 4
            for (int q = 0; q < 128; ++q) {
                const float* r = base + (size_t)q * EM_SREC;
                const float4 v = *reinterpret_cast<const float4*>(r + src);
                const float m = ysrc >= 0 ? r[ysrc] : 1.0f;
                acc[0] = fmaf(m, v.x, acc[0]); acc[1] = fmaf(m, v.y, acc[1]);
                acc[2] = fmaf(m, v.z, acc[2]); acc[3] = fmaf(m, v.w, acc[3]);
            }
        } else if (nout == 1) {
            const float* base = srec + (size_t)grp * 128 * EM_SREC + src;
            for (int q = 0; q < 128; ++q) acc[0] += base[(size_t)q * EM_SREC];
        }
        __syncthreads();
    }
#pragma unroll
    for (int k = 0; k < 4; ++k)
        if (k < nout) part[grp][out0 + k] = acc[k];
    __syncthreads();
    if (tid < EM_TOTAL) {
        const float v = (part[0][tid] + part[1][tid]) + (part[2][tid] + part[3][tid]);
        float* o = partial + (size_t)blockIdx.x * EM_TOTAL + tid;
        *o = accumulate ? *o + v : v;
    }
}

constexpr int WG_SPLITS = 37;
constexpr int WG_SPLITS_SIMT = 32;
constexpr int SM_SPLITS = 592;
constexpr int EM_SPLITS = 296;
constexpr int EM_SMEM = 2 * 256 * EM_SREC * (int)sizeof(float);

extern "C" int toued_lpg_wgrad_workspace_floats(void) {
    return WG_SPLITS * LPG_H * LPG_G + SM_SPLITS * SM_TOTAL + EM_SPLITS * EM_TOTAL;
}

extern "C" int toued_lpg_wgrad(const int32_t* obs, const uint8_t* done, const float* critic,
                               const float* lpg_params, const float* x, const float* h, const float* dgates,
                               const float* d_pi_hat, const float* dl, const float* dx, float* workspace,
                               int n_agents, int n_workers, int rollout_len, int obs_dim,
                               int lifetime_conditioning, int accumulate, void* stream) {
    const int R = n_agents * n_workers, L = rollout_len;
    TOUED_CHECK(R > 0 && L > 0, "toued_lpg_wgrad: empty problem");
    cudaStream_t st = (cudaStream_t)stream;
    const size_t ntok = (size_t)L * R;
    float* p_wh = workspace;
    float* p_sm = p_wh + (size_t)WG_SPLITS * LPG_H * LPG_G;
    float* p_em = p_sm + (size_t)SM_SPLITS * SM_TOTAL;
    {
        const size_t chunks = (ntok + WG_KC - 1) / WG_KC;
        const int cps = (int)((chunks + WG_SPLITS_SIMT - 1) / WG_SPLITS_SIMT);
        wgrad_wh_kernel<<<dim3(LPG_G / 64, LPG_H / 64, WG_SPLITS_SIMT), 256, 0, st>>>(done, h, dgates, p_wh, R, L, n_workers, cps, accumulate);
        TOUED_LAUNCH_CHECK();
    }
    {
        const int tps = (int)((ntok + SM_SPLITS - 1) / SM_SPLITS);
        wgrad_small_kernel<<<SM_SPLITS, 256, 0, st>>>(x, h, dgates, d_pi_hat, dl, p_sm, R, L, tps, accumulate);
        TOUED_LAUNCH_CHECK();
    }
    TOUED_CUDA(cudaFuncSetAttribute(embed_backward_kernel, cudaFuncAttributeMaxDynamicSharedMemorySize, EM_SMEM));
    embed_backward_kernel<<<EM_SPLITS, 256, EM_SMEM, st>>>(obs, done, critic, lpg_params, lpg_offsets(lifetime_conditioning ? 7 : 5).e_w0,
                                                      dx, p_em, nullptr, n_agents, n_workers, L, obs_dim, accumulate);
    TOUED_LAUNCH_CHECK();
    return 0;
}

__global__ void reduce_partials_kernel(const float* __restrict__ ws, float* __restrict__ grad, int X, int wh_splits, int sm_splits) {
    const LpgOffsets o = lpg_offsets(X);
    const float* p_wh = ws;
    const float* p_sm = p_wh + (size_t)WG_SPLITS * LPG_H * LPG_G;
    const float* p_em = p_sm + (size_t)SM_SPLITS * SM_TOTAL;
    const int i = blockIdx.x * blockDim.x + threadIdx.x;
    if (i < LPG_H * LPG_G) {
        float v = 0.f;
        for (int s = 0; s < wh_splits; ++s) v += p_wh[(size_t)s * LPG_H * LPG_G + i];
        grad[o.Wh + i] = v;
        return;
    }
    int k = i - LPG_H * LPG_G;
    if (k < SM_TOTAL) {
        float v = 0.f;
        for (int s = 0; s < sm_splits; ++s) v += p_sm[(size_t)s * SM_TOTAL + k];
        int dst;
        if (k < SM_BHN) { const int q = k / LPG_G, c = k % LPG_G; if (q == 7) dst = o.bi + c; else if (q < X) dst = o.Wi + q * LPG_G + c; else return; }
        else if (k < SM_WPI) dst = o.bhn + (k - SM_BHN);
        else if (k < SM_WY) dst = o.w_pi + (k - SM_WPI);
        else if (k < SM_BPI) dst = o.W_y + (k - SM_WY);
        else if (k < SM_BY) dst = o.b_pi;
        else dst = o.b_y + (k - SM_BY);
        grad[dst] = v;
        return;
    }
    k -= SM_TOTAL;
    if (k < EM_TOTAL) {
        float v = 0.f;
        for (int s = 0; s < EM_SPLITS; ++s) v += p_em[(size_t)s * EM_TOTAL + k];
        grad[o.e_w0 + k] = v;
    }
}

extern "C" int toued_lpg_wgrad_splits(int which) { return which == 0 ? WG_SPLITS_SIMT : SM_SPLITS; }

extern "C" int toued_lpg_wgrad_workspace_offset(int which) {
    if (which == 0) return 0;
    if (which == 1) return WG_SPLITS * LPG_H * LPG_G;
    return WG_SPLITS * LPG_H * LPG_G + SM_SPLITS * SM_TOTAL;
}

extern "C" int toued_lpg_wgrad_embed(const int32_t* obs, const uint8_t* done, const float* critic, const float* lpg_params,
                                     const float* dx, float* workspace, const uint32_t* cotangent_max, int n_agents,
                                     int n_workers, int rollout_len, int obs_dim, int lifetime_conditioning, int accumulate,
                                     void* stream) {
    float* p_em = workspace + toued_lpg_wgrad_workspace_offset(2);
    TOUED_CUDA(cudaFuncSetAttribute(embed_backward_kernel, cudaFuncAttributeMaxDynamicSharedMemorySize, EM_SMEM));
    embed_backward_kernel<<<EM_SPLITS, 256, EM_SMEM, (cudaStream_t)stream>>>(
        obs, done, critic, lpg_params, lpg_offsets(lifetime_conditioning ? 7 : 5).e_w0, dx, p_em, cotangent_max, n_agents,
        n_workers, rollout_len, obs_dim, accumulate);
    TOUED_LAUNCH_CHECK();
    return 0;
}

extern "C" int toued_reduce_partials(const float* workspace, float* grad, int lifetime_conditioning, int wh_splits,
                                     int sm_splits, void* stream) {
    const int n = LPG_H * LPG_G + SM_TOTAL + EM_TOTAL;
    TOUED_CHECK(wh_splits >= 1 && wh_splits <= WG_SPLITS, "toued_reduce_partials: wh_splits=%d out of range", wh_splits);
    TOUED_CHECK(sm_splits >= 1 && sm_splits <= SM_SPLITS, "toued_reduce_partials: sm_splits=%d out of range", sm_splits);
    reduce_partials_kernel<<<(n + 255) / 256, 256, 0, (cudaStream_t)stream>>>(workspace, grad, lifetime_conditioning ? 7 : 5, wh_splits, sm_splits);
    TOUED_LAUNCH_CHECK();
    return 0;
}

__global__ void adam_kernel(float* __restrict__ p, const float* __restrict__ g, float* __restrict__ m,
                            float* __restrict__ v, int n, float lr, float b1, float b2, float eps,
                            float c1, float c2) {
    const int i = blockIdx.x * blockDim.x + threadIdx.x;
    if (i >= n) return;
    const float gi = g[i];
    const float mi = b1 * m[i] + (1.0f - b1) * gi;
    const float vi = b2 * v[i] + (1.0f - b2) * gi * gi;
    m[i] = mi; v[i] = vi;
    p[i] -= lr * (mi / c1) / (sqrtf(vi / c2) + eps);
}

extern "C" int toued_adam(float* params, const float* grad, float* mu, float* nu, int n, int count,
                          float lr, float b1, float b2, float eps, void* stream) {
    TOUED_CHECK(n > 0 && count >= 1, "toued_adam: bad arguments");
    const float c1 = 1.0f - powf(b1, (float)count), c2 = 1.0f - powf(b2, (float)count);
    adam_kernel<<<(n + 255) / 256, 256, 0, (cudaStream_t)stream>>>(params, grad, mu, nu, n, lr, b1, b2, eps, c1, c2);
    TOUED_LAUNCH_CHECK();
    return 0;
}

__global__ void adam_dev_kernel(float* __restrict__ p, const float* __restrict__ g, float* __restrict__ m,
                                float* __restrict__ v, const int* __restrict__ count_dev, int n, float lr, float b1,
                                float b2, float eps) {
    const int i = blockIdx.x * blockDim.x + threadIdx.x;
    if (i >= n) return;
    const float cnt = (float)(*count_dev + 1);
    const float c1 = 1.0f - powf(b1, cnt), c2 = 1.0f - powf(b2, cnt);
    const float gi = g[i];
    const float mi = b1 * m[i] + (1.0f - b1) * gi;
    const float vi = b2 * v[i] + (1.0f - b2) * gi * gi;
    m[i] = mi; v[i] = vi;
    p[i] -= lr * (mi / c1) / (sqrtf(vi / c2) + eps);
}
__global__ void count_incr_kernel(int* count_dev) { *count_dev += 1; }

extern "C" int toued_adam_dev(float* params, const float* grad, float* mu, float* nu, int* count_dev, int n, float lr,
                              float b1, float b2, float eps, void* stream) {
    TOUED_CHECK(n > 0 && count_dev != nullptr, "toued_adam_dev: bad arguments");
    adam_dev_kernel<<<(n + 255) / 256, 256, 0, (cudaStream_t)stream>>>(params, grad, mu, nu, count_dev, n, lr, b1, b2, eps);
    TOUED_LAUNCH_CHECK();
    count_incr_kernel<<<1, 1, 0, (cudaStream_t)stream>>>(count_dev);
    TOUED_LAUNCH_CHECK();
    return 0;
}

__global__ void __launch_bounds__(1024) sqnorm_kernel(const float* __restrict__ g, int n, float* __restrict__ out) {
    __shared__ float part[32];
    float s = 0.f;
    for (int i = threadIdx.x; i < n; i += 1024) s = fmaf(g[i], g[i], s);
#pragma unroll
    for (int o = 16; o > 0; o >>= 1) s += __shfl_xor_sync(0xffffffffu, s, o);
    if ((threadIdx.x & 31) == 0) part[threadIdx.x >> 5] = s;
    __syncthreads();
    if (threadIdx.x < 32) {
        s = part[threadIdx.x];
#pragma unroll
        for (int o = 16; o > 0; o >>= 1) s += __shfl_xor_sync(0xffffffffu, s, o);
        if (threadIdx.x == 0) out[0] = s;
    }
}
__global__ void sgd_clip_kernel(float* __restrict__ p, const float* __restrict__ g, const float* __restrict__ sq, int n,
                                float lr, float max_norm) {
    const int i = blockIdx.x * blockDim.x + threadIdx.x;
    if (i >= n) return;
    const float norm = sqrtf(sq[0]);
    const float gi = norm < max_norm ? g[i] : (g[i] / norm) * max_norm;
    p[i] -= lr * gi;
}
extern "C" int toued_sgd_clip(float* params, const float* grad, float* sqnorm_scratch, int n, float lr, float max_norm,
                              void* stream) {
    TOUED_CHECK(n > 0 && sqnorm_scratch != nullptr, "toued_sgd_clip: bad arguments");
    sqnorm_kernel<<<1, 1024, 0, (cudaStream_t)stream>>>(grad, n, sqnorm_scratch);
    TOUED_LAUNCH_CHECK();
    sgd_clip_kernel<<<(n + 255) / 256, 256, 0, (cudaStream_t)stream>>>(params, grad, sqnorm_scratch, n, lr, max_norm);
    TOUED_LAUNCH_CHECK();
    return 0;
}

__global__ void cot_max_kernel(const float* __restrict__ d_pi_hat, const float* __restrict__ d_y_hat, size_t n_tok,
                               uint32_t* __restrict__ out_bits) {
    float m = 0.f;
    const size_t stride = (size_t)gridDim.x * blockDim.x;
    for (size_t i = (size_t)blockIdx.x * blockDim.x + threadIdx.x; i < n_tok; i += stride) m = fmaxf(m, fabsf(d_pi_hat[i]));
    const float4* y4 = reinterpret_cast<const float4*>(d_y_hat);
    for (size_t i = (size_t)blockIdx.x * blockDim.x + threadIdx.x; i < 2 * n_tok; i += stride) {
        const float4 v = y4[i];
        m = fmaxf(m, fmaxf(fmaxf(fabsf(v.x), fabsf(v.y)), fmaxf(fabsf(v.z), fabsf(v.w))));
    }
#pragma unroll
    for (int o = 16; o > 0; o >>= 1) m = fmaxf(m, __shfl_xor_sync(0xffffffffu, m, o));
    if ((threadIdx.x & 31) == 0 && m > 0.f) atomicMax(out_bits, __float_as_uint(m));
}

extern "C" int toued_cotangent_max(const float* d_pi_hat, const float* d_y_hat, int n_agents, int n_workers, int rollout_len,
                                   uint32_t* out_bits, void* stream) {
    const size_t n_tok = (size_t)n_agents * n_workers * rollout_len;
    TOUED_CHECK(n_tok > 0 && out_bits != nullptr, "toued_cotangent_max: bad arguments");
    cudaStream_t st = (cudaStream_t)stream;
    TOUED_CUDA(cudaMemsetAsync(out_bits, 0, sizeof(uint32_t), st));
    cot_max_kernel<<<296, 256, 0, st>>>(d_pi_hat, d_y_hat, n_tok, out_bits);
    TOUED_LAUNCH_CHECK();
    return 0;
}
```

to_ued_b200/csrc/lpg_common.cuh:

```cuda
#pragma once
#include "common.cuh"

constexpr int LPG_H = 256;
constexpr int LPG_Y = 8;
constexpr int LPG_E = 16;
constexpr int LPG_G = 3 * LPG_H;
constexpr int LPG_XP = 8;

struct LpgOffsets {
    int e_w0, e_b0, e_w1, e_b1, Wi, bi, Wh, bhn, w_pi, b_pi, W_y, b_y, total;
};
__host__ __device__ inline LpgOffsets lpg_offsets(int X) {
    LpgOffsets o; int p = 0;
    o.Wh = p; p += LPG_H * LPG_G;
    o.Wi = p; p += X * LPG_G;
    o.bi = p; p += LPG_G;
    o.bhn = p; p += LPG_H;
    o.w_pi = p; p += LPG_H;
    o.W_y = p; p += LPG_H * LPG_Y;
    o.b_y = p; p += LPG_Y;
    o.e_w0 = p; p += LPG_Y * LPG_E;
    o.e_b0 = p; p += LPG_E;
    o.e_w1 = p; p += LPG_E;
    o.e_b1 = p; p += 1;
    o.b_pi = p; p += 1;
    o.total = p;
    return o;
}

__device__ __forceinline__ float sigmoidf_(float x) { return 1.0f / (1.0f + __expf(-x)); }
__device__ __forceinline__ float tanhf_(float x) {
    const float e = __expf(2.0f * x);
    return 1.0f - 2.0f / (e + 1.0f);
}

__device__ __forceinline__ float ex2_approx(float x) { float y; asm("ex2.approx.ftz.f32 %0, %1;" : "=f"(y) : "f"(x)); return y; }
__device__ __forceinline__ float rcp_approx(float x) { float y; asm("rcp.approx.ftz.f32 %0, %1;" : "=f"(y) : "f"(x)); return y; }
__device__ __forceinline__ float tanh_mufu(float x) { float y; asm("tanh.approx.f32 %0, %1;" : "=f"(y) : "f"(x)); return y; }
__device__ __forceinline__ float sigmoid_mufu(float x) { return fmaf(0.5f, tanh_mufu(0.5f * x), 0.5f); }
__device__ __forceinline__ float sigmoid_fast(float x) { return rcp_approx(1.0f + ex2_approx(-1.4426950408889634f * x)); }
__device__ __forceinline__ float tanh_fast(float x) { return fmaf(2.0f, rcp_approx(1.0f + ex2_approx(-2.8853900817779268f * x)), -1.0f); }

template <int C>
__device__ __forceinline__ void softmax_c(const float (&z)[C], float (&p)[C]) {
    float m = z[0];
#pragma unroll
    for (int j = 1; j < C; ++j) m = fmaxf(m, z[j]);
    float s = 0.0f;
#pragma unroll
    for (int j = 0; j < C; ++j) { p[j] = __expf(z[j] - m); s += p[j]; }
    const float inv = 1.0f / s;
#pragma unroll
    for (int j = 0; j < C; ++j) p[j] *= inv;
}

template <int C>
__device__ __forceinline__ void tab_logits8(const float* table, int D, int32_t ob, float (&z)[C]) {
    const float tf = 0.001f * (float)ob_time(ob);
    const float4* row = reinterpret_cast<const float4*>(table + (size_t)ob_idx(ob) * 8);
    const float4* last = reinterpret_cast<const float4*>(table + (size_t)(D - 1) * 8);
    float r[8], l[8];
    const float4 a0 = row[0], a1 = row[1], b0 = last[0], b1 = last[1];
    r[0] = a0.x; r[1] = a0.y; r[2] = a0.z; r[3] = a0.w; r[4] = a1.x; r[5] = a1.y; r[6] = a1.z; r[7] = a1.w;
    l[0] = b0.x; l[1] = b0.y; l[2] = b0.z; l[3] = b0.w; l[4] = b1.x; l[5] = b1.y; l[6] = b1.z; l[7] = b1.w;
#pragma unroll
    for (int j = 0; j < C; ++j) z[j] = r[j] + tf * l[j];
}

__device__ __forceinline__ float block_sum(float v, float* red) {
#pragma unroll
    for (int o = 16; o > 0; o >>= 1) v += __shfl_xor_sync(0xffffffffu, v, o);
    const int lane = threadIdx.x & 31, warp = threadIdx.x >> 5, nw = (blockDim.x + 31) >> 5;
    __syncthreads();
    if (lane == 0) red[warp] = v;
    __syncthreads();
    float t = (lane < nw) ? red[lane] : 0.0f;
#pragma unroll
    for (int o = 16; o > 0; o >>= 1) t += __shfl_xor_sync(0xffffffffu, t, o);
    return t;
}
```

to_ued_b200/csrc/lpg_forward.cu:

```cuda
#include "lpg_common.cuh"
#include "tc.cuh"
#include "../../include/toued.h"

template <int E>
__device__ __forceinline__ void sort_cmpx(uint32_t& mine, uint32_t other, bool keep_min) {
    const uint32_t lo = min(mine, other), hi = max(mine, other);
    mine = keep_min ? lo : hi;
}

template <int E>
__global__ void __launch_bounds__(256)
sort_tokens_reg_kernel(const int32_t* __restrict__ obs, uint16_t* __restrict__ sorted_tok, int W, int L, int T) {
    constexpr int P2 = 256 * E;
    __shared__ uint32_t xch[P2];
    const int n = blockIdx.x, tid = threadIdx.x, base = tid * E;
    const int32_t* ob = obs + (size_t)n * (L + 1) * W;
    uint32_t v[E];
#pragma unroll
    for (int e = 0; e < E; ++e) {
        const int i = base + e;
        v[e] = i < T ? ((uint32_t)ob_idx(ob[i]) << 12) | (uint32_t)i : 0xFFFFFFFFu;
    }
    for (int k = 2; k <= P2; k <<= 1) {
        for (int j = k >> 1; j >= 32 * E; j >>= 1) {
#pragma unroll
            for (int e = 0; e < E; ++e) xch[base + e] = v[e];
            __syncthreads();
#pragma unroll
            for (int e = 0; e < E; ++e) {
                const int i = base + e;
                sort_cmpx<E>(v[e], xch[i ^ j], ((i & j) == 0) == ((i & k) == 0));
            }
            __syncthreads();
        }
        for (int j = min(k >> 1, 16 * E); j >= E; j >>= 1) {
            const int lane_mask = j / E;
#pragma unroll
            for (int e = 0; e < E; ++e) {
                const int i = base + e;
                const uint32_t other = __shfl_xor_sync(0xffffffffu, v[e], lane_mask);
                sort_cmpx<E>(v[e], other, ((i & j) == 0) == ((i & k) == 0));
            }
        }
#pragma unroll
        for (int j = E / 2; j > 0; j >>= 1) {
            if (j < k) {
#pragma unroll
                for (int e = 0; e < E; ++e) {
                    if ((e & j) == 0) {
                        const bool up = ((base + e) & k) == 0;
                        const uint32_t a = v[e], b = v[e | j];
                        const uint32_t lo = min(a, b), hi = max(a, b);
                        v[e] = up ? lo : hi;
                        v[e | j] = up ? hi : lo;
                    }
                }
            }
        }
    }
#pragma unroll
    for (int e = 0; e < E; ++e)
        if (base + e < T) sorted_tok[(size_t)n * T + base + e] = (uint16_t)(v[e] & 0xFFFu);
}

__global__ void __launch_bounds__(256)
sort_tokens_kernel(const int32_t* __restrict__ obs, uint16_t* __restrict__ sorted_tok,
                   int W, int L, int T, int P2) {
    extern __shared__ uint32_t keys[];
    const int n = blockIdx.x;
    const int32_t* ob = obs + (size_t)n * (L + 1) * W;
    for (int i = threadIdx.x; i < P2; i += blockDim.x)
        keys[i] = i < T ? ((uint32_t)ob_idx(ob[i]) << 12) | (uint32_t)i : 0xFFFFFFFFu;
    __syncthreads();
    for (int k = 2; k <= P2; k <<= 1) {
        for (int j = k >> 1; j > 0; j >>= 1) {
            for (int i = threadIdx.x; i < P2; i += blockDim.x) {
                const int ixj = i ^ j;
                if (ixj > i) {
                    const uint32_t a = keys[i], b = keys[ixj];
                    const bool up = (i & k) == 0;
                    if ((a > b) == up) { keys[i] = b; keys[ixj] = a; }
                }
            }
            __syncthreads();
        }
    }
    for (int i = threadIdx.x; i < T; i += blockDim.x)
        sorted_tok[(size_t)n * T + i] = (uint16_t)(keys[i] & 0xFFFu);
}

extern "C" int toued_sort_tokens(const int32_t* obs, uint16_t* sorted_tok, int n_agents, int n_workers,
                                 int rollout_len, void* stream) {
    const int T = n_workers * rollout_len;
    TOUED_CHECK(T > 0 && T <= 4096, "toued_sort_tokens: W*L=%d must be in 1..4096", T);
    int P2 = 1; while (P2 < T) P2 <<= 1;
    cudaStream_t st = (cudaStream_t)stream;
    switch (P2) {
        case 512:  sort_tokens_reg_kernel<2><<<n_agents, 256, 0, st>>>(obs, sorted_tok, n_workers, rollout_len, T); break;
        case 1024: sort_tokens_reg_kernel<4><<<n_agents, 256, 0, st>>>(obs, sorted_tok, n_workers, rollout_len, T); break;
        case 2048: sort_tokens_reg_kernel<8><<<n_agents, 256, 0, st>>>(obs, sorted_tok, n_workers, rollout_len, T); break;
        case 4096: sort_tokens_reg_kernel<16><<<n_agents, 256, 0, st>>>(obs, sorted_tok, n_workers, rollout_len, T); break;
        default:   sort_tokens_kernel<<<n_agents, 256, P2 * sizeof(uint32_t), st>>>(obs, sorted_tok, n_workers, rollout_len, T, P2);
    }
    TOUED_LAUNCH_CHECK();
    return 0;
}

__device__ __forceinline__ void embed_mlp2(const float (&y0)[LPG_Y], const float (&y1)[LPG_Y],
                                           const float* __restrict__ sp, float& out0, float& out1) {
    out0 = out1 = sp[LPG_Y * LPG_E + LPG_E + LPG_E];
#pragma unroll 4
    for (int e = 0; e < LPG_E; ++e) {
        float a0 = sp[LPG_Y * LPG_E + e], a1 = a0;
#pragma unroll
        for (int i = 0; i < LPG_Y; ++i) {
            const float wgt = sp[i * LPG_E + e];
            a0 = fmaf(y0[i], wgt, a0);
            a1 = fmaf(y1[i], wgt, a1);
        }
        const float w1 = sp[LPG_Y * LPG_E + LPG_E + e];
        out0 = fmaf(fmaxf(a0, 0.0f), w1, out0);
        out1 = fmaf(fmaxf(a1, 0.0f), w1, out1);
    }
}

__global__ void __launch_bounds__(256, 4)
lpg_prepare_kernel(const int32_t* __restrict__ obs, const uint8_t* __restrict__ action,
                   const float* __restrict__ reward, const uint8_t* __restrict__ done,
                   const float* __restrict__ actor, const float* __restrict__ critic,
                   const float* __restrict__ lpg, const int32_t* __restrict__ step,
                   const LevelRec* __restrict__ levels, float* __restrict__ x, unsigned char* __restrict__ ximg,
                   int n_agents, int W, int L, int D, int cond, int emb_off, int lpg_stride) {
    __shared__ float sp_s[LPG_Y * LPG_E + LPG_E + LPG_E + 1];
    if (lpg_stride == 0) {
        for (int i = threadIdx.x; i < LPG_Y * LPG_E + 2 * LPG_E + 1; i += blockDim.x) sp_s[i] = lpg[emb_off + i];
        __syncthreads();
    }
    const size_t g = (size_t)blockIdx.x * blockDim.x + threadIdx.x;
    const size_t total = (size_t)n_agents * L * W;
    if (g >= total) return;
    const int w = (int)(g % W);
    const int t = (int)((g / W) % L);
    const int n = (int)(g / ((size_t)W * L));
    const float* sp = lpg_stride ? lpg + (size_t)n * lpg_stride + emb_off : sp_s;
    const int32_t ob = obs[((size_t)n * (L + 1) + t) * W + w];
    const int32_t ob1 = obs[((size_t)n * (L + 1) + t + 1) * W + w];
    const float* at = actor + (size_t)n * D * 8;
    const float* ct = critic + (size_t)n * D * 8;
    float z[TOUED_NUM_ACTIONS], p[TOUED_NUM_ACTIONS];
    tab_logits8<TOUED_NUM_ACTIONS>(at, D, ob, z);
    softmax_c<TOUED_NUM_ACTIONS>(z, p);
    const int a = action[g];
    float pa = p[0];
#pragma unroll
    for (int j = 1; j < TOUED_NUM_ACTIONS; ++j) pa = (a == j) ? p[j] : pa;
    float zy[LPG_Y], y0[LPG_Y], y1[LPG_Y];
    tab_logits8<LPG_Y>(ct, D, ob, zy);
    softmax_c<LPG_Y>(zy, y0);
    tab_logits8<LPG_Y>(ct, D, ob1, zy);
    softmax_c<LPG_Y>(zy, y1);
    const float d = done[g] ? 1.0f : 0.0f;
    float pyt, pyt1;
    embed_mlp2(y0, y1, sp, pyt, pyt1);
    pyt1 *= (1.0f - d);
    const size_t row = (size_t)n * W + w;
    float4* xo = reinterpret_cast<float4*>(x + ((size_t)t * n_agents * W + row) * LPG_XP);
    xo[0] = make_float4(reward[g], d, pa + 1e-8f, pyt);
    const float4 v1 = make_float4(pyt1, cond ? (float)step[n] : 0.0f, cond ? (float)levels[n].lifetime : 0.0f, 1.0f);
    xo[1] = v1;
    if (ximg) {
        const size_t Rp = ((size_t)n_agents * W + 63) & ~(size_t)63;
        __half2 b0 = __floats2half2_rn(reward[g], d), b1 = __floats2half2_rn(pa + 1e-8f, pyt);
        __half2 b2 = __floats2half2_rn(v1.x, v1.y), b3 = __floats2half2_rn(v1.z, v1.w);
        uint4 pk;
        pk.x = *reinterpret_cast<uint32_t*>(&b0); pk.y = *reinterpret_cast<uint32_t*>(&b1);
        pk.z = *reinterpret_cast<uint32_t*>(&b2); pk.w = *reinterpret_cast<uint32_t*>(&b3);
        *reinterpret_cast<uint4*>(ximg + tile_img_offset((size_t)t * Rp + row, 1, 0)) = pk;
    }
}

extern "C" int toued_lpg_prepare(const int32_t* obs, const uint8_t* action, const float* reward,
                                 const uint8_t* done, const float* actor, const float* critic,
                                 const float* lpg_params, const int32_t* step, const void* levels,
                                 float* x, void* ximg, int n_agents, int n_workers, int rollout_len, int obs_dim,
                                 int lifetime_conditioning, int lpg_stride, void* stream) {
    const size_t total = (size_t)n_agents * rollout_len * n_workers;
    TOUED_CHECK(total > 0, "toued_lpg_prepare: empty problem");
    lpg_prepare_kernel<<<(unsigned)((total + 255) / 256), 256, 0, (cudaStream_t)stream>>>(
        obs, action, reward, done, actor, critic, lpg_params, step, (const LevelRec*)levels, x, (unsigned char*)ximg,
        n_agents, n_workers, rollout_len, obs_dim, lifetime_conditioning,
        lpg_offsets(lifetime_conditioning ? 7 : 5).e_w0, lpg_stride);
    TOUED_LAUNCH_CHECK();
    return 0;
}

constexpr int GF_TM = 64;
constexpr int GF_KC = 16;
constexpr int GF_HS = LPG_H + 4;

__device__ __forceinline__ void cp_async16(void* smem, const void* gmem) {
    asm volatile("cp.async.cg.shared.global [%0], [%1], 16;" ::"r"(smem_u32(smem)), "l"(gmem));
}
__device__ __forceinline__ void cp_async_commit() { asm volatile("cp.async.commit_group;"); }
template <int N> __device__ __forceinline__ void cp_async_wait() { asm volatile("cp.async.wait_group %0;" ::"n"(N)); }

template <int X>
__global__ void __launch_bounds__(256, 1)
gru_forward_kernel(const float* __restrict__ x, const uint8_t* __restrict__ done,
                   const float* __restrict__ lpg_base, float* __restrict__ h_out, float* __restrict__ gates,
                   float* __restrict__ pi_hat, float* __restrict__ y_hat, int R, int L, int W, int lpg_stride) {
    const float* lpg = lpg_base + (size_t)((blockIdx.x * 64) / W) * lpg_stride;
    extern __shared__ __align__(16) float sm[];
    float* hA = sm;
    float* hB = hA + GF_TM * GF_HS;
    float* Bs = hB + GF_TM * GF_HS;
    float* sWi = Bs + 2 * GF_KC * 192;
    float* sbi = sWi + X * LPG_G;
    float* sbhn = sbi + LPG_G;
    float* swp = sbhn + LPG_H;
    float* sWy = swp + LPG_H;
    float* sx = sWy + LPG_H * LPG_Y;
    __shared__ float sdone[GF_TM];
    const LpgOffsets o = lpg_offsets(X);
    const float* Wh = lpg + o.Wh;
    const int tid = threadIdx.x;
    const int row0 = blockIdx.x * GF_TM;
    const int nrows = min(GF_TM, R - row0);

    for (int i = tid; i < X * LPG_G; i += 256) sWi[i] = lpg[o.Wi + i];
    for (int i = tid; i < LPG_G; i += 256) sbi[i] = lpg[o.bi + i];
    for (int i = tid; i < LPG_H; i += 256) { sbhn[i] = lpg[o.bhn + i]; swp[i] = lpg[o.w_pi + i]; }
    for (int i = tid; i < LPG_H * LPG_Y; i += 256) sWy[i] = lpg[o.W_y + i];
    for (int i = tid; i < GF_TM * GF_HS; i += 256) hB[i] = 0.0f;
    const float b_pi = lpg[o.b_pi];
    float b_y[LPG_Y];
#pragma unroll
    for (int i = 0; i < LPG_Y; ++i) b_y[i] = lpg[o.b_y + i];
    __syncthreads();

    const int rg = tid >> 4;
    const int jg = tid & 15;

    for (int t = L - 1; t >= 0; --t) {
        { float* tmp = hA; hA = hB; hB = tmp; }
        if (tid < GF_TM) {
            const int r = row0 + tid;
            sdone[tid] = (tid < nrows && done[((size_t)(r / W) * L + t) * W + (r % W)]) ? 1.0f : 0.0f;
        }
        for (int i = tid; i < GF_TM * 2; i += 256) {
            const int r = i >> 1;
            float4 v = make_float4(0.f, 0.f, 0.f, 0.f);
            if (r < nrows) v = reinterpret_cast<const float4*>(x + ((size_t)t * R + row0 + r) * LPG_XP)[i & 1];
            reinterpret_cast<float4*>(sx + r * LPG_XP)[i & 1] = v;
        }
        __syncthreads();
        for (int i = tid; i < GF_TM * 64; i += 256) {
            const int r = i >> 6;
            if (sdone[r] != 0.0f) reinterpret_cast<float4*>(hA + r * GF_HS)[i & 63] = make_float4(0.f, 0.f, 0.f, 0.f);
        }
        __syncthreads();

        for (int jb = 0; jb < 4; ++jb) {
            float acc[4][4][3];
#pragma unroll
            for (int i = 0; i < 4; ++i)
#pragma unroll
                for (int j = 0; j < 4; ++j) { acc[i][j][0] = 0.f; acc[i][j][1] = 0.f; acc[i][j][2] = 0.f; }
            auto load_chunk = [&](int buf, int k0) {
#pragma unroll
                for (int q = 0; q < 3; ++q) {
                    const int f = tid + q * 256;
                    const int kk = f / 48, rem = f % 48, gte = rem >> 4, c4 = rem & 15;
                    cp_async16(Bs + (buf * GF_KC + kk) * 192 + gte * 64 + c4 * 4,
                               Wh + (size_t)(k0 + kk) * LPG_G + gte * LPG_H + jb * 64 + c4 * 4);
                }
                cp_async_commit();
            };
            load_chunk(0, 0);
            for (int kc = 0; kc < LPG_H / GF_KC; ++kc) {
                if (kc + 1 < LPG_H / GF_KC) { load_chunk((kc + 1) & 1, (kc + 1) * GF_KC); cp_async_wait<1>(); }
                else cp_async_wait<0>();
                __syncthreads();
                const float* bs = Bs + (kc & 1) * GF_KC * 192;
#pragma unroll
                for (int k4 = 0; k4 < GF_KC; k4 += 4) {
                    float4 a[4];
#pragma unroll
                    for (int i = 0; i < 4; ++i)
                        a[i] = *reinterpret_cast<const float4*>(hA + (rg * 4 + i) * GF_HS + kc * GF_KC + k4);
#pragma unroll
                    for (int kk = 0; kk < 4; ++kk) {
                        float4 b[3];
#pragma unroll
                        for (int gte = 0; gte < 3; ++gte)
                            b[gte] = *reinterpret_cast<const float4*>(bs + (k4 + kk) * 192 + gte * 64 + jg * 4);
#pragma unroll
                        for (int i = 0; i < 4; ++i) {
                            const float av = kk == 0 ? a[i].x : kk == 1 ? a[i].y : kk == 2 ? a[i].z : a[i].w;
#pragma unroll
                            for (int gte = 0; gte < 3; ++gte) {
                                acc[i][0][gte] = fmaf(av, b[gte].x, acc[i][0][gte]);
                                acc[i][1][gte] = fmaf(av, b[gte].y, acc[i][1][gte]);
                                acc[i][2][gte] = fmaf(av, b[gte].z, acc[i][2][gte]);
                                acc[i][3][gte] = fmaf(av, b[gte].w, acc[i][3][gte]);
                            }
                        }
                    }
                }
                __syncthreads();
            }
            const int j0 = jb * 64 + jg * 4;
#pragma unroll
            for (int i = 0; i < 4; ++i) {
                const int rl = rg * 4 + i;
                float xr[X];
#pragma unroll
                for (int q = 0; q < X; ++q) xr[q] = sx[rl * LPG_XP + q];
                float hn4[4], r4[4], z4[4], n4[4], hv[4];
#pragma unroll
                for (int j = 0; j < 4; ++j) {
                    const int u = j0 + j;
                    float gr = sbi[u], gz = sbi[LPG_H + u], gn = sbi[2 * LPG_H + u];
#pragma unroll
                    for (int q = 0; q < X; ++q) {
                        gr = fmaf(xr[q], sWi[q * LPG_G + u], gr);
                        gz = fmaf(xr[q], sWi[q * LPG_G + LPG_H + u], gz);
                        gn = fmaf(xr[q], sWi[q * LPG_G + 2 * LPG_H + u], gn);
                    }
                    const float rr = sigmoidf_(gr + acc[i][j][0]);
                    const float zz = sigmoidf_(gz + acc[i][j][1]);
                    const float hn = acc[i][j][2] + sbhn[u];
                    const float nn = tanhf_(gn + rr * hn);
                    const float hp = hA[rl * GF_HS + u];
                    r4[j] = rr; z4[j] = zz; n4[j] = nn; hn4[j] = hn;
                    hv[j] = (1.0f - zz) * nn + zz * hp;
                }
                *reinterpret_cast<float4*>(hB + rl * GF_HS + j0) = make_float4(hv[0], hv[1], hv[2], hv[3]);
                if (rl < nrows) {
                    const size_t base = ((size_t)t * R + row0 + rl) * LPG_H + j0;
                    *reinterpret_cast<float4*>(h_out + base) = make_float4(hv[0], hv[1], hv[2], hv[3]);
                    if (gates) {
                        const size_t gs = (size_t)L * R * LPG_H;
                        *reinterpret_cast<float4*>(gates + base) = make_float4(r4[0], r4[1], r4[2], r4[3]);
                        *reinterpret_cast<float4*>(gates + gs + base) = make_float4(z4[0], z4[1], z4[2], z4[3]);
                        *reinterpret_cast<float4*>(gates + 2 * gs + base) = make_float4(n4[0], n4[1], n4[2], n4[3]);
                        *reinterpret_cast<float4*>(gates + 3 * gs + base) = make_float4(hn4[0], hn4[1], hn4[2], hn4[3]);
                    }
                }
            }
        }
        __syncthreads();
        {
            const int rl = tid >> 2, part = tid & 3;
            float hacc[1 + LPG_Y];
#pragma unroll
            for (int c = 0; c < 1 + LPG_Y; ++c) hacc[c] = 0.0f;
            for (int k = part * 64; k < part * 64 + 64; ++k) {
                const float yv = fmaxf(hB[rl * GF_HS + k], 0.0f);
                hacc[0] = fmaf(yv, swp[k], hacc[0]);
#pragma unroll
                for (int c = 0; c < LPG_Y; ++c) hacc[1 + c] = fmaf(yv, sWy[k * LPG_Y + c], hacc[1 + c]);
            }
#pragma unroll
            for (int c = 0; c < 1 + LPG_Y; ++c) {
                hacc[c] += __shfl_xor_sync(0xffffffffu, hacc[c], 1);
                hacc[c] += __shfl_xor_sync(0xffffffffu, hacc[c], 2);
            }
            if (part == 0 && rl < nrows) {
                const size_t tok = (size_t)t * R + row0 + rl;
                pi_hat[tok] = hacc[0] + b_pi;
                float zl[LPG_Y], pr[LPG_Y];
#pragma unroll
                for (int c = 0; c < LPG_Y; ++c) zl[c] = hacc[1 + c] + b_y[c];
                softmax_c<LPG_Y>(zl, pr);
                float4* yo = reinterpret_cast<float4*>(y_hat + tok * LPG_Y);
                yo[0] = make_float4(pr[0], pr[1], pr[2], pr[3]);
                yo[1] = make_float4(pr[4], pr[5], pr[6], pr[7]);
            }
        }
    }
}

static size_t gru_fwd_smem(int X) {
    return sizeof(float) * (2 * GF_TM * GF_HS + 2 * GF_KC * 192 + X * LPG_G + LPG_G + 2 * LPG_H +
                            LPG_H * LPG_Y + GF_TM * LPG_XP);
}

extern "C" int toued_gru_forward(const float* x, const uint8_t* done, const float* lpg_params, float* h_out,
                                 float* gates, float* pi_hat, float* y_hat, int n_agents, int n_workers,
                                 int rollout_len, int lifetime_conditioning, int lpg_stride, void* stream) {
    const int R = n_agents * n_workers;
    TOUED_CHECK(R > 0 && rollout_len > 0, "toued_gru_forward: empty problem");
    TOUED_CHECK(lpg_stride == 0 || n_workers % 64 == 0, "toued_gru_forward: per-agent parameters need n_workers %% 64 == 0");
    const int blocks = (R + GF_TM - 1) / GF_TM;
    cudaStream_t st = (cudaStream_t)stream;
    if (lifetime_conditioning) {
        const size_t smem = gru_fwd_smem(7);
        TOUED_CUDA(cudaFuncSetAttribute(gru_forward_kernel<7>, cudaFuncAttributeMaxDynamicSharedMemorySize, (int)smem));
        gru_forward_kernel<7><<<blocks, 256, smem, st>>>(x, done, lpg_params, h_out, gates, pi_hat, y_hat, R, rollout_len, n_workers, lpg_stride);
    } else {
        const size_t smem = gru_fwd_smem(5);
        TOUED_CUDA(cudaFuncSetAttribute(gru_forward_kernel<5>, cudaFuncAttributeMaxDynamicSharedMemorySize, (int)smem));
        gru_forward_kernel<5><<<blocks, 256, smem, st>>>(x, done, lpg_params, h_out, gates, pi_hat, y_hat, R, rollout_len, n_workers, lpg_stride);
    }
    TOUED_LAUNCH_CHECK();
    return 0;
}
```

to_ued_b200/meta/train.py:

```python
from __future__ import annotations

from typing import Any, Optional

import numpy as np
import torch

from .. import _lib
from ..util import prng
from ..util.data import AgentState, LpgHyperparams
from ..agents.lpg_agent import Tape, train_lpg_agent, train_lpg_agent_steps
from ..agents.agents import eval_agent
from ..environments.gridworld.gridworld import EnvState


class LPGTrainState:

    def __init__(self, model, params, tx, opt_state=None, step=0):
        self.model, self.params, self.tx = model, params, tx
        self.opt_state = tx.init(params) if opt_state is None else opt_state
        self.step = step

    def replace(self, **kw):
        d = dict(model=self.model, params=self.params, tx=self.tx, opt_state=self.opt_state, step=self.step)
        d.update(kw)
        return LPGTrainState(**d)


class MetaGradWorkspace:

    def __init__(self, n_agents, n_workers, rollout_len, obs_dim, num_updates, n_params, device):
        N, W, L, K = n_agents, n_workers, rollout_len, num_updates
        R = N * W
        f32 = torch.float32
        self.tape = Tape(N, W, L, obs_dim, K, device, keep_gates=True)
        self.d_pi_hat2 = [torch.empty((L, R), dtype=f32, device=device) for _ in range(2)]
        self.d_y_hat2 = [torch.empty((L, R, 8), dtype=f32, device=device) for _ in range(2)]
        self.dx2 = [torch.empty((L, R, 2), dtype=f32, device=device) for _ in range(2)]
        self.d_pi_hat, self.d_y_hat, self.dx = self.d_pi_hat2[0], self.d_y_hat2[0], self.dx2[0]
        self.dl2 = [torch.empty((L, R, 8), dtype=f32, device=device) for _ in range(2)]
        self.dl = self.dl2[0]
        self.lam = torch.empty((N, obs_dim, 8), dtype=f32, device=device)
        self.mu = torch.empty((N, obs_dim, 8), dtype=f32, device=device)
        self.whT = torch.empty((768, 256), dtype=f32, device=device)
        self.partials = torch.empty(_lib.lib().toued_lpg_wgrad_workspace_floats(), dtype=f32, device=device)
        self.loss_scal = torch.empty((N, 2), dtype=f32, device=device)
        self.ab_scratch = torch.empty(_lib.lib().toued_agent_scratch_floats(N, W, L, obs_dim), dtype=f32, device=device)
        if self.tape.precision == "tc":
            Rp = (R + 63) // 64 * 64
            self.whb_img = torch.empty(256 * 768, dtype=torch.float16, device=device)
            self.cotmax = torch.zeros(K, dtype=torch.int32, device=device)
            self.dgimg2 = [torch.zeros(L * Rp * 1024 * 2, dtype=torch.uint8, device=device) for _ in range(2)]
            self.dgimg = self.dgimg2[0]
        self.off_small = _lib.lib().toued_lpg_wgrad_workspace_offset(1)
        self.key = (N, W, L, obs_dim, K, n_params, str(device))


_WS_CACHE = {}
_STREAMS = {}


def _workspace(n, w, L, D, K, P, device, slot=0) -> MetaGradWorkspace:
    import to_ued_b200
    key = (n, w, L, D, K, P, str(device), to_ued_b200.GRU_PRECISION)
    if _WS_CACHE and next(iter(_WS_CACHE))[:-1] != key:
        _WS_CACHE.clear()
    ws = _WS_CACHE.get(key + (slot,))
    if ws is None:
        ws = _WS_CACHE[key + (slot,)] = MetaGradWorkspace(n, w, L, D, K, P, device)
    return ws


def _eval_stream(device):
    key = ("eval", str(device))
    if key not in _STREAMS:
        _STREAMS[key] = [torch.cuda.Stream(device=device)]
    return _STREAMS[key][0]


def _side_streams(device, n):
    key = str(device)
    lst = _STREAMS.setdefault(key, [])
    while len(lst) < n:
        lst.append(torch.cuda.Stream(device=device))
    return lst[:n]


def _world():
    import torch.distributed as dist
    if dist.is_available() and dist.is_initialized():
        return dist.get_world_size(), dist
    return 1, None


def lpg_meta_grad_train_step(rng, lpg_train_state: LPGTrainState, agent_states: AgentState, value_critic_states,
                             rollout_manager, num_mini_batches: int, gamma: float, gae_lambda: float,
                             lpg_hypers: LpgHyperparams, *, outer_product_quirk: bool = True,
                             global_agent_offset: int = 0, global_num_agents: Optional[int] = None,
                             eval_workers: int = 4, return_grad: bool = False, num_streams: Optional[int] = None,
                             _static: Optional[dict] = None):
    env = rollout_manager.env
    actor, critic = agent_states.actor_state, agent_states.critic_state
    N, W = agent_states.env_state.packed.shape
    L, K, D = rollout_manager.train_rollout_len, lpg_hypers.num_agent_updates, env.obs_dim
    dev = actor.params.device
    world, dist = _world()
    n_global = global_num_agents if global_num_agents is not None else N * world
    if dist is not None and global_num_agents is None:
        global_agent_offset = dist.get_rank() * N
    model = lpg_train_state.model
    cond = int(model.lifetime_conditioning)
    lpg = lpg_train_state.params
    P = lpg.numel()
    p, s = _lib.ptr, _lib.stream_ptr()

    rngs = prng.split_device(prng.to_device(rng, dev), n_global, global_agent_offset, N)[0]
    r_train, r_eval, r_evalagent = prng.chain_device(rngs, 3)

    if N % num_mini_batches != 0:
        raise ValueError(f"local agents ({N}) must be divisible by num_mini_batches ({num_mini_batches})")
    nb = N // num_mini_batches
    import to_ued_b200
    if num_streams is None:
        num_streams = to_ued_b200.NUM_STREAMS
    S = max(1, min(int(num_streams), num_mini_batches))
    wss = [_workspace(nb, W, L, D, K, P, dev, slot=i) for i in range(S)]
    main = torch.cuda.current_stream()
    streams = [main] if S == 1 else _side_streams(dev, S)
    tc = wss[0].tape.precision == "tc"
    gscale = 1.0 / n_global
    bK = [c / K for c in (lpg_hypers.policy_entropy_coeff, lpg_hypers.target_entropy_coeff,
                          lpg_hypers.policy_l2_coeff, lpg_hypers.target_l2_coeff)]
    if _static is not None:
        new_actor, new_critic, new_step, new_state, new_obs = _static["out"]
    else:
        new_actor = torch.empty_like(actor.params)
        new_critic = torch.empty_like(critic.params)
        new_step = torch.empty_like(actor.step)
        new_state = torch.empty_like(agent_states.env_state.packed)
        new_obs = torch.empty_like(agent_states.env_obs)
    msums = [torch.zeros(8, dtype=torch.float32, device=dev) for _ in range(S)]
    returns = torch.empty(N, dtype=torch.float32, device=dev)
    ready = torch.cuda.Event()
    ready.record(main)

    def _phase(label, chunk, stream):
        if to_ued_b200.PHASE_EVENTS is not None:
            e = torch.cuda.Event(enable_timing=True)
            e.record(stream)
            to_ued_b200.PHASE_EVENTS.append((label, chunk, e))
    _phase("start", -1, main)
    eval_done = [None] * S
    eval_stream = _side_streams(dev, S + 1)[S] if S > 1 else _eval_stream(dev)
    pool = _side_streams(dev, 5 * S + 1)
    ab_streams, em_streams = pool[S + 1:2 * S + 1], pool[2 * S + 1:3 * S + 1]
    ev_streams = [eval_stream] + pool[3 * S + 1:4 * S]
    wg_streams = pool[4 * S + 1:5 * S + 1]
    if not to_ued_b200.SIDE_STREAMS:
        ab_streams = em_streams = ev_streams = wg_streams = list(streams)
    evs = {}

    ctx, gens = {}, {}

    def forward_begin(mb):
        slot = mb % S
        ws, tape = wss[slot], wss[slot].tape
        with torch.cuda.stream(streams[slot]):
            if S > 1 and mb < S:
                streams[slot].wait_event(ready)
            if eval_done[slot] is not None:
                streams[slot].wait_event(eval_done[slot])
            sl = slice(mb * nb, (mb + 1) * nb)
            sub = AgentState(actor.replace(params=actor.params[sl], step=actor.step[sl]),
                             critic.replace(params=critic.params[sl], step=critic.step[sl]),
                             _sub_level(agent_states.level, sl), agent_states.env_obs[sl],
                             EnvState(agent_states.env_state.packed[sl], env.max_n_objs))
            levels = sub.level.packed
            gens[mb] = (train_lpg_agent_steps(r_train[sl], lpg_train_state, sub, rollout_manager, K,
                                              lpg_hypers.agent_target_coeff, tape=tape), sl, levels)
            next(gens[mb][0])

    def forward_step(mb):
        with torch.cuda.stream(streams[mb % S]):
            try:
                next(gens[mb][0])
            except StopIteration as fin:
                gens[mb] = (fin.value,) + gens[mb][1:]
            _phase("update", mb, streams[mb % S])

    def forward_end(mb):
        slot = mb % S
        ws, tape = wss[slot], wss[slot].tape
        res, sl, levels = gens.pop(mb)
        with torch.cuda.stream(streams[slot]):
            s = _lib.stream_ptr()
            if not isinstance(res, tuple):
                try:
                    while True:
                        next(res)
                except StopIteration as fin:
                    res = fin.value
            sub2, _, am = res
            state = sub2.env_state.packed
            _lib.call("toued_rollout", p(levels), p(r_eval[sl]), p(tape.actor[K]), None, p(state), p(tape.obs[K]),
                      p(tape.action[K]), p(tape.reward[K]), p(tape.done[K]), None, nb, W, L, D,
                      env.max_grid_size, env.max_n_objs, 0, s)
            _lib.call("toued_sort_tokens", p(tape.obs[K]), p(tape.sorted_tok[K]), nb, W, L, s)
            fwd_done = torch.cuda.Event()
            fwd_done.record(streams[slot])
            _phase("forward", mb, streams[slot])
            with torch.cuda.stream(ev_streams[slot]):
                ev_streams[slot].wait_event(fwd_done)
                returns[sl] = eval_agent(r_evalagent[sl], rollout_manager, levels, tape.actor[K], eval_workers)
                eval_done[slot] = torch.cuda.Event()
                eval_done[slot].record(ev_streams[slot])
            ctx[mb] = (sl, sub2, state, am, levels)

    def backward_begin(mb):
        slot = mb % S
        ws, tape = wss[slot], wss[slot].tape
        sl = ctx[mb][0]
        with torch.cuda.stream(streams[slot]):
            s = _lib.stream_ptr()
            if mb < S:
                if tc:
                    _lib.call("toued_pack_wh_backward", p(lpg), p(ws.whb_img), s)
                else:
                    _lib.call("toued_transpose_wh", p(lpg), p(ws.whT), s)
            vparams = value_critic_states.params[sl]
            _lib.call("toued_meta_loss", p(tape.obs[K]), p(tape.action[K]), p(tape.reward[K]), p(tape.done[K]),
                      p(tape.sorted_tok[K]), p(vparams), p(tape.actor[K]), p(ws.lam), p(ws.mu), p(ws.loss_scal),
                      nb, W, L, D, vparams.shape[-1], float(gamma), float(gae_lambda), float(gscale),
                      int(outer_product_quirk), s)
            evs[mb] = {"ml": torch.cuda.Event(), "ab": {}, "bwd": {}, "wg": {}, "em": {}}
            evs[mb]["ml"].record(streams[slot])

    def _agent_backward(ws, tape, k, buf, s):
        _lib.call("toued_agent_backward", p(tape.obs[k]), p(tape.action[k]), p(tape.sorted_tok[k]),
                  p(tape.pi_hat[k]), p(tape.y_hat[k]), p(tape.actor[k]), p(tape.critic[k]),
                  p(tape.actor[k + 1]), p(tape.critic[k + 1]), p(tape.scalars[k]), p(ws.lam), p(ws.mu),
                  p(ws.d_pi_hat2[buf]), p(ws.d_y_hat2[buf]), nb, W, L, D, float(actor.learning_rate),
                  float(critic.learning_rate), float(actor.max_grad_norm),
                  float(lpg_hypers.agent_target_coeff), *[float(b) for b in bK], float(gscale), p(ws.ab_scratch), s)

    def backward_step(mb, k):
        slot = mb % S
        ws, tape = wss[slot], wss[slot].tape
        first = (mb < S and k == K - 1)
        if not tc:
            with torch.cuda.stream(streams[slot]):
                s = _lib.stream_ptr()
                _agent_backward(ws, tape, k, 0, s)
                _lib.call("toued_gru_backward", p(tape.done[k]), p(lpg), p(ws.whT), p(tape.h[k]), p(tape.gates[k]),
                          p(tape.y_hat[k]), p(ws.d_pi_hat), p(ws.d_y_hat), p(ws.dl), p(ws.dx), nb, W, L, cond, s)
                _lib.call("toued_lpg_wgrad", p(tape.obs[k]), p(tape.done[k]), p(tape.critic[k]), p(lpg), p(tape.x[k]),
                          p(tape.h[k]), p(tape.gates[k]), p(ws.d_pi_hat), p(ws.dl), p(ws.dx), p(ws.partials),
                          nb, W, L, D, cond, 0 if first else 1, s)
            return
        ev, buf = evs[mb], k & 1
        for d in ("ab", "bwd", "wg", "em"):
            ev[d][k] = torch.cuda.Event()
        with torch.cuda.stream(ab_streams[slot]):
            st = ab_streams[slot]
            if k == K - 1:
                st.wait_event(ev["ml"])
            if k + 2 <= K - 1:
                st.wait_event(ev["wg"][k + 2])
            _agent_backward(ws, tape, k, buf, _lib.stream_ptr())
            _lib.call("toued_cotangent_max", p(ws.d_pi_hat2[buf]), p(ws.d_y_hat2[buf]), nb, W, L, p(ws.cotmax[k:k + 1]),
                      _lib.stream_ptr())
            ev["ab"][k].record(st)
        with torch.cuda.stream(streams[slot]):
            st = streams[slot]
            s = _lib.stream_ptr()
            st.wait_event(ev["ab"][k])
            if k + 2 <= K - 1:
                st.wait_event(ev["em"][k + 2])
                st.wait_event(ev["wg"][k + 2])
            _lib.call("toued_gru_backward_tc", p(tape.done[k]), p(lpg), p(ws.whb_img), p(tape.h16[k]),
                      p(tape.fac[k]), p(tape.y_hat[k]), p(ws.d_pi_hat2[buf]), p(ws.d_y_hat2[buf]), p(ws.dgimg2[buf]), p(ws.dl2[buf]),
                      p(ws.dx2[buf]), p(ws.cotmax[k:k + 1]), nb, W, L, cond, s)
            ev["bwd"][k].record(st)
            _phase(f"bwd{k}", mb, st)
        with torch.cuda.stream(wg_streams[slot]):
            st = wg_streams[slot]
            st.wait_event(ev["bwd"][k])
            _lib.call("toued_lpg_wgrad_tc", p(tape.hpimg[k]), p(ws.dgimg2[buf]), p(tape.ximg[k]), p(tape.h16[k]),
                      p(ws.d_pi_hat2[buf]), p(ws.dl2[buf]), p(ws.partials), p(ws.partials[ws.off_small:]),
                      p(ws.cotmax[k:k + 1]), nb, W, L, 0 if first else 1, _lib.stream_ptr())
            ev["wg"][k].record(st)
            _phase(f"wgrad{k}", mb, st)
        with torch.cuda.stream(em_streams[slot]):
            st = em_streams[slot]
            st.wait_event(ev["bwd"][k])
            _lib.call("toued_lpg_wgrad_embed", p(tape.obs[k]), p(tape.done[k]), p(tape.critic[k]), p(lpg),
                      p(ws.dx2[buf]), p(ws.partials), p(ws.cotmax[k:k + 1]), nb, W, L, D, cond, 0 if first else 1,
                      _lib.stream_ptr())
            ev["em"][k].record(st)

    def backward_end(mb):
        slot = mb % S
        ws, tape, msum = wss[slot], wss[slot].tape, msums[slot]
        sl, sub2, state, am, levels = ctx.pop(mb)
        with torch.cuda.stream(streams[slot]):
            ev = evs.pop(mb)
            if ev["em"]:
                streams[slot].wait_event(ev["em"][0])
                streams[slot].wait_event(ev["wg"][0])
            lpg_loss, value_loss = ws.loss_scal[:, 0], ws.loss_scal[:, 1]
            reg = (lpg_loss - lpg_hypers.policy_entropy_coeff * am.policy_entropy + lpg_hypers.policy_l2_coeff * am.policy_l2
                   - lpg_hypers.target_entropy_coeff * am.critic_entropy + lpg_hypers.target_l2_coeff * am.critic_l2)
            msum[:7] += torch.stack([lpg_loss.sum(), reg.sum(), value_loss.sum(), am.policy_l2.sum(),
                                     am.policy_entropy.sum(), am.critic_loss.sum(), am.critic_l2.sum()])
            msum[7] += am.critic_entropy.sum()
            new_actor[sl] = sub2.actor_state.params
            new_critic[sl] = sub2.critic_state.params
            new_step[sl] = sub2.actor_state.step
            new_state[sl] = state
            new_obs[sl] = tape.obs[K][:, -1]
            _phase("reverse_end", mb, streams[slot])

    for g0 in range(0, num_mini_batches, S):
        group = range(g0, min(num_mini_batches, g0 + S))
        for mb in group:
            forward_begin(mb)
            forward_step(mb)
        for k in range(1, K):
            for mb in group:
                forward_step(mb)
        for mb in group:
            forward_end(mb)
        for mb in group:
            backward_begin(mb)
        for k in reversed(range(K)):
            for mb in group:
                backward_step(mb, k)
        for mb in group:
            backward_end(mb)
    for st in ([] if S == 1 else list(streams)) + ev_streams:
        ev = torch.cuda.Event()
        ev.record(st)
        main.wait_event(ev)
    s = _lib.stream_ptr()
    msum = msums[0] if S == 1 else torch.stack(msums).sum(0)

    grad = torch.empty(P, dtype=torch.float32, device=dev)
    L_ = _lib.lib()
    n_wh, n_sm = (L_.toued_wgrad_tc_splits(), L_.toued_wgrad_tc_small_splits()) if tc else \
        (L_.toued_lpg_wgrad_splits(0), L_.toued_lpg_wgrad_splits(1))
    _lib.call("toued_reduce_partials", p(wss[0].partials), p(grad), cond, n_wh, n_sm, s)
    for ws in wss[1:min(S, num_mini_batches)]:
        g2 = torch.empty_like(grad)
        _lib.call("toued_reduce_partials", p(ws.partials), p(g2), cond, n_wh, n_sm, s)
        grad += g2
    red = torch.cat([grad, msum, returns.sum().view(1)])
    if dist is not None:
        dist.all_reduce(red)
    grad, mvec = red[:P], red[P:] / n_global
    if _static is not None:
        ost = lpg_train_state.opt_state
        lpg_train_state.tx.update_dev_(lpg, grad, ost["mu"], ost["nu"], _static["count_dev"])
        new_lpg = lpg_train_state
    else:
        new_params = lpg.clone()
        opt_state = lpg_train_state.tx.update_(new_params, grad, {**lpg_train_state.opt_state,
                                                                  "mu": lpg_train_state.opt_state["mu"].clone(),
                                                                  "nu": lpg_train_state.opt_state["nu"].clone()})
        new_lpg = lpg_train_state.replace(params=new_params, opt_state=opt_state, step=lpg_train_state.step + 1)
    agent_out = agent_states.replace(
        actor_state=actor.replace(params=new_actor, step=new_step),
        critic_state=critic.replace(params=new_critic, step=new_step if _static is not None else new_step.clone()),
        env_obs=new_obs, env_state=EnvState(new_state, env.max_n_objs),
        host_step=_advance_host_step(agent_states.host_step, agent_states.level.lifetime, K))
    if _static is not None:
        value_critic_states.step.add_(K + 1)
        value_out = value_critic_states
    else:
        value_out = value_critic_states.replace(step=value_critic_states.step + (K + 1))
    metrics = {
        "lpg_loss": mvec[0], "reg_lpg_loss": mvec[1], "value_loss": mvec[2],
        "lpg_agent": {"policy_l2": mvec[3], "policy_entropy": mvec[4], "critic_loss": mvec[5],
                      "critic_l2": mvec[6], "critic_entropy": mvec[7]},
        "lpg_agent_return": mvec[8],
    }
    if return_grad:
        metrics["_grad"] = grad
    if _static is not None:
        metrics["_mvec"] = mvec
    _phase("end", -1, main)
    return new_lpg, agent_out, value_out, metrics


def _advance_host_step(step, lifetime, k):
    if step is None:
        return None
    return np.minimum(step + k, np.maximum(step, lifetime)).astype(np.int32)


def _sub_level(level, sl):
    from ..util.data import Level
    return Level(level.env_params, level.lifetime[sl], level.buffer_id[sl], level.packed[sl])
```

Baseline: 472.4 million.

## Record per-token softmax outputs in forward and reuse them in backward kernels

The LPG prepare kernel and the agent update now store per-token policy and critic softmax rows (tok_p, tok_y, tok_p1, tok_y1) on the tape. The agent backward, wgrad and embed-backward kernels load these rows instead of recomputing table logits and softmax from the actor/critic tables. The agent backward also caches lam/mu rows in shared memory so they are not reloaded from global memory in the second run pass. This trades recomputation for extra global memory traffic and tape storage of about 8 floats per token per record, which may cost more on a bandwidth-bound path.

After: 472.0 million, median of 6. Within noise of the previous version (-0.1%).

```diff
diff --git a/include/toued.h b/include/toued.h
--- a/include/toued.h
+++ b/include/toued.h
@@ -31,6 +31,11 @@
                       const float* lpg_params, const int32_t* step, const void* levels, float* x,
                       void* ximg, int n_agents, int n_workers, int rollout_len, int obs_dim,
                       int lifetime_conditioning, int lpg_stride, void* stream);
+int toued_lpg_prepare_rec(const int32_t* obs, const uint8_t* action, const float* reward,
+                          const uint8_t* done, const float* actor, const float* critic,
+                          const float* lpg_params, const int32_t* step, const void* levels, float* x,
+                          void* ximg, float* tok_p, float* tok_y, int n_agents, int n_workers, int rollout_len,
+                          int obs_dim, int lifetime_conditioning, int lpg_stride, void* stream);
 
 int toued_gru_forward(const float* x, const uint8_t* done, const float* lpg_params, float* h_out,
                       float* gates, float* pi_hat, float* y_hat, int n_agents, int n_workers,
@@ -38,7 +43,8 @@
 
 int toued_agent_scratch_floats(int n_agents, int n_workers, int rollout_len, int obs_dim);
 int toued_agent_update(const int32_t* obs, const uint8_t* action, const uint16_t* sorted_tok,
-                       const float* pi_hat, const float* y_hat, const float* actor_in,
+                       const float* pi_hat, const float* y_hat, const float* tok_p, const float* tok_y,
+                       float* tok_p1, float* tok_y1, const float* actor_in,
                        const float* critic_in, float* actor_out, float* critic_out,
                        const void* levels, int32_t* step, float* scalars, int n_agents,
                        int n_workers, int rollout_len, int obs_dim, float lr_actor, float lr_critic,
@@ -53,8 +59,8 @@
                     float gae_lambda, float grad_scale, int outer_product_quirk, void* stream);
 
 int toued_agent_backward(const int32_t* obs, const uint8_t* action, const uint16_t* sorted_tok,
-                         const float* pi_hat, const float* y_hat, const float* actor_k,
-                         const float* critic_k, const float* actor_k1, const float* critic_k1,
+                         const float* pi_hat, const float* y_hat, const float* tok_p,
+                         const float* tok_y, const float* tok_p1, const float* tok_y1,
                          const float* update_scalars, float* lam, float* mu, float* d_pi_hat,
                          float* d_y_hat, int n_agents, int n_workers, int rollout_len, int obs_dim,
                          float lr_actor, float lr_critic, float max_grad_norm,
@@ -70,15 +76,14 @@
                        int rollout_len, int lifetime_conditioning, void* stream);
 
 int toued_lpg_wgrad_workspace_floats(void);
-int toued_lpg_wgrad(const int32_t* obs, const uint8_t* done, const float* critic,
-                    const float* lpg_params, const float* x, const float* h, const float* dgates,
-                    const float* d_pi_hat, const float* dl, const float* dx, float* workspace,
-                    int n_agents, int n_workers, int rollout_len, int obs_dim,
+int toued_lpg_wgrad(const float* tok_y, const uint8_t* done, const float* lpg_params, const float* x,
+                    const float* h, const float* dgates, const float* d_pi_hat, const float* dl,
+                    const float* dx, float* workspace, int n_agents, int n_workers, int rollout_len,
                     int lifetime_conditioning, int accumulate, void* stream);
 int toued_lpg_wgrad_workspace_offset(int which);
-int toued_lpg_wgrad_embed(const int32_t* obs, const uint8_t* done, const float* critic, const float* lpg_params,
-                          const float* dx, float* workspace, const uint32_t* cotangent_max, int n_agents, int n_workers,
-                          int rollout_len, int obs_dim, int lifetime_conditioning, int accumulate, void* stream);
+int toued_lpg_wgrad_embed(const float* tok_y, const uint8_t* done, const float* lpg_params, const float* dx,
+                          float* workspace, const uint32_t* cotangent_max, int n_agents, int n_workers,
+                          int rollout_len, int lifetime_conditioning, int accumulate, void* stream);
 int toued_lpg_wgrad_splits(int which);
 int toued_reduce_partials(const float* workspace, float* grad, int lifetime_conditioning, int wh_splits,
                           int sm_splits, void* stream);
diff --git a/to_ued_b200/_lib.py b/to_ued_b200/_lib.py
--- a/to_ued_b200/_lib.py
+++ b/to_ued_b200/_lib.py
@@ -34,19 +34,20 @@
     "toued_env_reset": [_P] * 3 + [_I] * 3 + [_P],
     "toued_sort_tokens": [_P] * 2 + [_I] * 3 + [_P],
     "toued_lpg_prepare": [_P] * 11 + [_I] * 6 + [_P],
+    "toued_lpg_prepare_rec": [_P] * 13 + [_I] * 6 + [_P],
     "toued_gru_forward": [_P] * 7 + [_I] * 5 + [_P],
-    "toued_agent_update": [_P] * 12 + [_I] * 4 + [_F] * 4 + [_I, _P, _P],
+    "toued_agent_update": [_P] * 16 + [_I] * 4 + [_F] * 4 + [_I, _P, _P],
     "toued_agent_scratch_floats": [_I] * 4,
     "toued_meta_loss": [_P] * 10 + [_I] * 5 + [_F] * 3 + [_I, _P],
     "toued_agent_backward": [_P] * 14 + [_I] * 4 + [_F] * 9 + [_P, _P],
     "toued_transpose_wh": [_P] * 3,
     "toued_gru_backward": [_P] * 10 + [_I] * 4 + [_P],
     "toued_lpg_wgrad_workspace_floats": [],
-    "toued_lpg_wgrad": [_P] * 11 + [_I] * 6 + [_P],
+    "toued_lpg_wgrad": [_P] * 10 + [_I] * 5 + [_P],
     "toued_reduce_partials": [_P, _P, _I, _I, _I, _P],
     "toued_lpg_wgrad_splits": [_I],
     "toued_lpg_wgrad_workspace_offset": [_I],
-    "toued_lpg_wgrad_embed": [_P] * 7 + [_I] * 6 + [_P],
+    "toued_lpg_wgrad_embed": [_P] * 6 + [_I] * 5 + [_P],
     "toued_cotangent_max": [_P, _P, _I, _I, _I, _P, _P],
     "toued_pack_wh_backward": [_P] * 3,
     "toued_gru_backward_tc": [_P] * 12 + [_I] * 4 + [_P],
diff --git a/to_ued_b200/agents/lpg_agent.py b/to_ued_b200/agents/lpg_agent.py
--- a/to_ued_b200/agents/lpg_agent.py
+++ b/to_ued_b200/agents/lpg_agent.py
@@ -64,6 +64,10 @@
             self.gates = torch.empty((ka, 4, L, R, 256), dtype=f32, device=dev) if self.record else None
         self.pi_hat = torch.empty((ka, L, R), dtype=f32, device=dev)
         self.y_hat = torch.empty((ka, L, R, 8), dtype=f32, device=dev)
+        self.tok_p = torch.empty((ka, N, L, W, 8), dtype=f32, device=dev)
+        self.tok_y = torch.empty((ka, N, L + 1, W, 8), dtype=f32, device=dev)
+        self.tok_p1 = torch.empty((ka, N, L, W, 8), dtype=f32, device=dev) if self.record else None
+        self.tok_y1 = torch.empty((ka, N, L, W, 8), dtype=f32, device=dev) if self.record else None
         self.scalars = torch.empty((ka, N, 8), dtype=f32, device=dev)
         self.scal_sum = torch.zeros((N, 8), dtype=f32, device=dev)
         self.step_in = torch.empty((ka, N), dtype=i32, device=dev)
@@ -124,9 +128,9 @@
         ev_sort.record(side)
     _mark("rollout")
     tape.step_in[a].copy_(step)
-    _lib.call("toued_lpg_prepare", p(tape.obs[r]), p(tape.action[r]), p(tape.reward[r]), p(tape.done[r]),
+    _lib.call("toued_lpg_prepare_rec", p(tape.obs[r]), p(tape.action[r]), p(tape.reward[r]), p(tape.done[r]),
               p(tape.actor[t0]), p(tape.critic[t0]), p(lpg_params), p(step), p(levels), p(tape.x[a]),
-              p(tape.ximg[a]) if tape.ximg is not None else None,
+              p(tape.ximg[a]) if tape.ximg is not None else None, p(tape.tok_p[a]), p(tape.tok_y[a]),
               N, W, L, D, int(lifetime_conditioning), int(lpg_stride), s)
     if lpg_stride and tape.precision == "tc":
         _lib.call("toued_gru_forward_tc_multi", p(tape.x[a]), p(tape.done[r]), p(lpg_params), p(tape.wh_img),
@@ -144,7 +148,8 @@
     cur.wait_event(ev_sort)
     _mark("sort_wait")
     _lib.call("toued_agent_update", p(tape.obs[r]), p(tape.action[r]), p(tape.sorted_tok[r]), p(tape.pi_hat[a]),
-              p(tape.y_hat[a]), p(tape.actor[t0]), p(tape.critic[t0]), p(tape.actor[t1]), p(tape.critic[t1]),
+              p(tape.y_hat[a]), p(tape.tok_p[a]), p(tape.tok_y[a]), p(tape.tok_p1[a]) if tape.record else None,
+              p(tape.tok_y1[a]) if tape.record else None, p(tape.actor[t0]), p(tape.critic[t0]), p(tape.actor[t1]), p(tape.critic[t1]),
               p(levels), p(step), p(tape.scalars[a]), N, W, L, D, float(lr_actor), float(lr_critic),
               float(max_grad_norm), float(agent_target_coeff), int(precopied), p(tape.agent_scratch), s)
     tape.scal_sum += tape.scalars[a]
diff --git a/to_ued_b200/csrc/agent_backward.cu b/to_ued_b200/csrc/agent_backward.cu
--- a/to_ued_b200/csrc/agent_backward.cu
+++ b/to_ued_b200/csrc/agent_backward.cu
@@ -134,13 +134,10 @@
 
 struct TokFwd { float p[5], y[8], pa, q, tf; int a; };
 
-__device__ __forceinline__ TokFwd tok_forward(const float* at, const float* ct, int D, int32_t o, int a) {
+__device__ __forceinline__ TokFwd tok_record(const float* prow, const float* yrow, int32_t o, int a) {
     TokFwd f;
-    float z[5], zy[8];
-    tab_logits8<5>(at, D, o, z);
-    softmax_c<5>(z, f.p);
-    tab_logits8<8>(ct, D, o, zy);
-    softmax_c<8>(zy, f.y);
+    load_row8(prow, f.p);
+    load_row8(yrow, f.y);
     f.a = a;
     f.pa = f.p[0];
 #pragma unroll
@@ -173,9 +170,9 @@
 __global__ void __launch_bounds__(256, 2)
 agent_backward_kernel(const int32_t* __restrict__ obs, const uint8_t* __restrict__ action,
                       const uint16_t* __restrict__ sorted_tok, const float* __restrict__ pi_hat,
-                      const float* __restrict__ y_hat, const float* __restrict__ actor_k,
-                      const float* __restrict__ critic_k, const float* __restrict__ actor_k1,
-                      const float* __restrict__ critic_k1, const float* __restrict__ upd_scal,
+                      const float* __restrict__ y_hat, const float* __restrict__ tok_p,
+                      const float* __restrict__ tok_y, const float* __restrict__ tok_p1,
+                      const float* __restrict__ tok_y1, const float* __restrict__ upd_scal,
                       float* lam, float* mu, float* __restrict__ d_pi_hat, float* __restrict__ d_y_hat,
                       float* run_scratch, int n_agents, int W, int L, int D, float lr_a, float lr_c, float max_norm,
                       float alpha, float b_pent, float b_yent, float b_pl2, float b_yl2, float gscale) {
@@ -188,10 +185,10 @@
     const int32_t* ob = obs + (size_t)n * (L + 1) * W;
     const uint8_t* act = action + (size_t)n * T;
     const uint16_t* st = sorted_tok + (size_t)n * T;
-    const float* a0 = actor_k + (size_t)n * D * 8;
-    const float* c0 = critic_k + (size_t)n * D * 8;
-    const float* a1 = actor_k1 + (size_t)n * D * 8;
-    const float* c1 = critic_k1 + (size_t)n * D * 8;
+    const float* pk = tok_p + (size_t)n * T * 8;
+    const float* yk = tok_y + (size_t)n * (L + 1) * W * 8;
+    const float* pk1 = tok_p1 + (size_t)n * T * 8;
+    const float* yk1 = tok_y1 + (size_t)n * T * 8;
     float* lm = lam + (size_t)n * D * 8;
     float* mm = mu + (size_t)n * D * 8;
     const float invT = 1.0f / (float)T;
@@ -205,7 +202,7 @@
 #pragma unroll
     for (int j = 0; j < 13; ++j) last[j] = 0.f;
     for (int tok = tid; tok < T; tok += 256) {
-        const TokFwd f = tok_forward(a1, c1, D, ob[tok], act[tok]);
+        const TokFwd f = tok_record(pk1 + (size_t)tok * 8, yk1 + (size_t)tok * 8, ob[tok], act[tok]);
         float* r = rec + tok * 13;
         {
             float dh[5], s = 0.f;
@@ -266,7 +263,7 @@
     for (int tok = tid; tok < T; tok += 256) {
         const int t = tok / W, w = tok - t * W;
         const size_t li = (size_t)t * R + (size_t)n * W + w;
-        const TokFwd f = tok_forward(a0, c0, D, ob[tok], act[tok]);
+        const TokFwd f = tok_record(pk + (size_t)tok * 8, yk + (size_t)tok * 8, ob[tok], act[tok]);
         float yh[8]; load8(y_hat + li * 8, yh);
         float* r = rec + tok * 13;
         tok_grad(f, pi_hat[li], yh, invT, alpha, r);
@@ -283,10 +280,11 @@
         const float* g = runv + r * 13;
         float l8[8], m8[8];
         load8(lm + (size_t)row * 8, l8); load8(mm + (size_t)row * 8, m8);
-#pragma unroll
-        for (int j = 0; j < 5; ++j) dot_a = fmaf(g[j], l8[j], dot_a);
-#pragma unroll
-        for (int j = 0; j < 8; ++j) dot_c = fmaf(g[5 + j], m8[j], dot_c);
+        float* lr = rec + r * 13;
+#pragma unroll
+        for (int j = 0; j < 5; ++j) { dot_a = fmaf(g[j], l8[j], dot_a); lr[j] = l8[j]; }
+#pragma unroll
+        for (int j = 0; j < 8; ++j) { dot_c = fmaf(g[5 + j], m8[j], dot_c); lr[5 + j] = m8[j]; }
     }
     dot_a = block_sum(dot_a, red); dot_c = block_sum(dot_c, red);
     float ll[8], ml[8];
@@ -310,14 +308,12 @@
     for (int j = 0; j < 13; ++j) wl[j] = s_wlast[j];
 
     for (int r = tid; r < si.nruns; r += 256) {
-        const int row = si.run_row[r];
         float* g = runv + r * 13;
-        float l8[8], m8[8];
-        load8(lm + (size_t)row * 8, l8); load8(mm + (size_t)row * 8, m8);
-#pragma unroll
-        for (int j = 0; j < 5; ++j) g[j] = ka * (l8[j] - pa_ * g[j]);
-#pragma unroll
-        for (int j = 0; j < 8; ++j) g[5 + j] = kc * (m8[j] - pc_ * g[5 + j]);
+        const float* lr = rec + r * 13;
+#pragma unroll
+        for (int j = 0; j < 5; ++j) g[j] = ka * (lr[j] - pa_ * g[j]);
+#pragma unroll
+        for (int j = 0; j < 8; ++j) g[5 + j] = kc * (lr[5 + j] - pc_ * g[5 + j]);
     }
     __syncthreads();
     float hl[13];
@@ -327,7 +323,7 @@
         const int tok = si.tok[pos];
         const int t = tok / W, w = tok - t * W;
         const size_t li = (size_t)t * R + (size_t)n * W + w;
-        const TokFwd f = tok_forward(a0, c0, D, ob[tok], act[tok]);
+        const TokFwd f = tok_record(pk + (size_t)tok * 8, yk + (size_t)tok * 8, ob[tok], act[tok]);
         const float ph = pi_hat[li];
         float yh[8]; load8(y_hat + li * 8, yh);
         float* r = rec + tok * 13;
@@ -395,8 +391,8 @@
 }
 
 extern "C" int toued_agent_backward(const int32_t* obs, const uint8_t* action, const uint16_t* sorted_tok,
-                                    const float* pi_hat, const float* y_hat, const float* actor_k,
-                                    const float* critic_k, const float* actor_k1, const float* critic_k1,
+                                    const float* pi_hat, const float* y_hat, const float* tok_p,
+                                    const float* tok_y, const float* tok_p1, const float* tok_y1,
                                     const float* update_scalars, float* lam, float* mu, float* d_pi_hat,
                                     float* d_y_hat, int n_agents, int n_workers, int rollout_len, int obs_dim,
                                     float lr_actor, float lr_critic, float max_grad_norm,
@@ -406,13 +402,14 @@
     const int T = n_workers * rollout_len;
     TOUED_CHECK(n_agents > 0 && T > 0, "toued_agent_backward: empty problem");
     TOUED_CHECK(run_scratch != nullptr, "toued_agent_backward: run_scratch (toued_agent_scratch_floats) is required");
+    TOUED_CHECK(tok_p && tok_y && tok_p1 && tok_y1, "toued_agent_backward: the token-forward records are required");
     const size_t smem = sizeof(float) * ((size_t)T * 13 + 2 * 256 * 13) + seg_index_bytes(T);
     TOUED_CHECK(smem <= 200 * 1024, "toued_agent_backward: W*L=%d too large for shared memory", T);
     TOUED_CUDA(cudaFuncSetAttribute(agent_backward_kernel, cudaFuncAttributeMaxDynamicSharedMemorySize, (int)smem));
     TOUED_CUDA(cudaFuncSetAttribute(agent_backward_kernel, cudaFuncAttributePreferredSharedMemoryCarveout, 100));
     cudaStream_t st = (cudaStream_t)stream;
     agent_backward_kernel<<<n_agents, 256, smem, st>>>(
-        obs, action, sorted_tok, pi_hat, y_hat, actor_k, critic_k, actor_k1, critic_k1, update_scalars, lam, mu,
+        obs, action, sorted_tok, pi_hat, y_hat, tok_p, tok_y, tok_p1, tok_y1, update_scalars, lam, mu,
         d_pi_hat, d_y_hat, run_scratch, n_agents, n_workers, rollout_len, obs_dim, lr_actor, lr_critic, max_grad_norm,
         agent_target_coeff, policy_entropy_coeff, target_entropy_coeff, policy_l2_coeff, target_l2_coeff, grad_scale);
     TOUED_LAUNCH_CHECK();
diff --git a/to_ued_b200/csrc/agent_update.cu b/to_ued_b200/csrc/agent_update.cu
--- a/to_ued_b200/csrc/agent_update.cu
+++ b/to_ued_b200/csrc/agent_update.cu
@@ -7,8 +7,10 @@
 __global__ void __launch_bounds__(256, 2)
 agent_update_kernel(const int32_t* __restrict__ obs, const uint8_t* __restrict__ action,
                     const uint16_t* __restrict__ sorted_tok, const float* __restrict__ pi_hat,
-                    const float* __restrict__ y_hat, const float* __restrict__ actor_in,
-                    const float* __restrict__ critic_in, float* actor_out, float* critic_out,
+                    const float* __restrict__ y_hat, const float* __restrict__ tok_p,
+                    const float* __restrict__ tok_y, float* __restrict__ tok_p1, float* __restrict__ tok_y1,
+                    const float* __restrict__ actor_in, const float* __restrict__ critic_in, float* actor_out,
+                    float* critic_out,
                     const LevelRec* __restrict__ levels, int32_t* __restrict__ step,
                     float* __restrict__ scal, float* run_scratch, int n_agents, int W, int L, int D,
                     float lr_a, float lr_c, float max_norm, float alpha, int tables_precopied) {
@@ -27,6 +29,8 @@
     float* a_out = actor_out + (size_t)n * D * 8;
     float* c_out = critic_out + (size_t)n * D * 8;
     const float invT = 1.0f / (float)T;
+    const float* pk = tok_p + (size_t)n * T * 8;
+    const float* yk = tok_y + (size_t)n * (L + 1) * W * 8;
     const SegIndex si = seg_index_build(idxmem, iscan, sorted_tok + (size_t)n * T, ob, T);
 
     if (!tables_precopied)
@@ -43,11 +47,9 @@
         const int t = tok / W, w = tok - t * W;
         const size_t li = (size_t)t * R + (size_t)n * W + w;
         const int32_t o = ob[tok];
-        float z[5], p[5], zy[8], y[8];
-        tab_logits8<5>(a_in, D, o, z);
-        softmax_c<5>(z, p);
-        tab_logits8<8>(c_in, D, o, zy);
-        softmax_c<8>(zy, y);
+        float p[5], y[8];
+        load_row8(pk + (size_t)tok * 8, p);
+        load_row8(yk + (size_t)tok * 8, y);
         const int a = act[tok];
         float pa = p[0];
 #pragma unroll
@@ -128,6 +130,10 @@
         softmax_c<5>(z, p);
         tab_logits8<8>(c_out, D, o, zy);
         softmax_c<8>(zy, y);
+        if (tok_p1) {
+            store_row8(tok_p1 + ((size_t)n * T + tok) * 8, p);
+            store_row8(tok_y1 + ((size_t)n * T + tok) * 8, y);
+        }
 #pragma unroll
         for (int j = 0; j < 5; ++j) { const float q = p[j] + 1e-8f; ea -= q * logf(q); }
 #pragma unroll
@@ -150,7 +156,8 @@
 }
 
 extern "C" int toued_agent_update(const int32_t* obs, const uint8_t* action, const uint16_t* sorted_tok,
-                                  const float* pi_hat, const float* y_hat, const float* actor_in,
+                                  const float* pi_hat, const float* y_hat, const float* tok_p, const float* tok_y,
+                                  float* tok_p1, float* tok_y1, const float* actor_in,
                                   const float* critic_in, float* actor_out, float* critic_out,
                                   const void* levels, int32_t* step, float* scalars, int n_agents,
                                   int n_workers, int rollout_len, int obs_dim, float lr_actor,
@@ -164,9 +171,11 @@
     TOUED_CUDA(cudaFuncSetAttribute(agent_update_kernel, cudaFuncAttributeMaxDynamicSharedMemorySize, (int)smem));
     TOUED_CUDA(cudaFuncSetAttribute(agent_update_kernel, cudaFuncAttributePreferredSharedMemoryCarveout, 100));
     TOUED_CHECK(run_scratch != nullptr, "toued_agent_update: run_scratch (toued_agent_scratch_floats) is required");
+    TOUED_CHECK(tok_p != nullptr && tok_y != nullptr, "toued_agent_update: the token-forward record (tok_p, tok_y) is required");
+    TOUED_CHECK((tok_p1 == nullptr) == (tok_y1 == nullptr), "toued_agent_update: tok_p1 and tok_y1 go together");
     cudaStream_t st = (cudaStream_t)stream;
     agent_update_kernel<<<n_agents, 256, smem, st>>>(
-        obs, action, sorted_tok, pi_hat, y_hat, actor_in, critic_in, actor_out, critic_out,
+        obs, action, sorted_tok, pi_hat, y_hat, tok_p, tok_y, tok_p1, tok_y1, actor_in, critic_in, actor_out, critic_out,
         (const LevelRec*)levels, step, scalars, run_scratch, n_agents, n_workers, rollout_len, obs_dim,
         lr_actor, lr_critic, max_grad_norm, agent_target_coeff, tables_precopied);
     TOUED_LAUNCH_CHECK();
diff --git a/to_ued_b200/csrc/lpg_backward.cu b/to_ued_b200/csrc/lpg_backward.cu
--- a/to_ued_b200/csrc/lpg_backward.cu
+++ b/to_ued_b200/csrc/lpg_backward.cu
@@ -326,10 +326,10 @@
 constexpr int EM_TOTAL = LPG_Y * LPG_E + 2 * LPG_E + 1;
 constexpr int EM_SREC = 44;
 __global__ void __launch_bounds__(256, 2)
-embed_backward_kernel(const int32_t* __restrict__ obs, const uint8_t* __restrict__ done,
-                      const float* __restrict__ critic, const float* __restrict__ lpg, int emb_off,
+embed_backward_kernel(const float* __restrict__ tok_y, const uint8_t* __restrict__ done,
+                      const float* __restrict__ lpg, int emb_off,
                       const float* __restrict__ dx, float* __restrict__ partial, const uint32_t* __restrict__ cotmax,
-                      int n_agents, int W, int L, int D, int accumulate) {
+                      int n_agents, int W, int L, int accumulate) {
     __shared__ float sp[EM_TOTAL];
     __shared__ float part[4][EM_TOTAL + 3];
     const float inv_s = cotmax ? 1.0f / cot_scale_from_max(*cotmax) : 1.0f;
@@ -357,12 +357,9 @@
             for (int i = 0; i < 8; ++i) y[s][i] = 0.f;
         if (ok) {
             const int w = (int)(g % W), t = (int)((g / W) % L), n = (int)(g / ((size_t)W * L));
-            const float* ct = critic + (size_t)n * D * 8;
-            float zy[8];
-            tab_logits8<8>(ct, D, obs[((size_t)n * (L + 1) + t) * W + w], zy);
-            softmax_c<8>(zy, y[0]);
-            tab_logits8<8>(ct, D, obs[((size_t)n * (L + 1) + t + 1) * W + w], zy);
-            softmax_c<8>(zy, y[1]);
+            const float* yr = tok_y + (((size_t)n * (L + 1) + t) * W + w) * 8;
+            load_row8(yr, y[0]);
+            load_row8(yr + (size_t)W * 8, y[1]);
             const float2 d = *reinterpret_cast<const float2*>(dx + ((size_t)t * R + (size_t)n * W + w) * 2);
             dp[0] = d.x * inv_s;
             dp[1] = done[g] ? 0.0f : d.y * inv_s;
@@ -435,10 +432,9 @@
     return WG_SPLITS * LPG_H * LPG_G + SM_SPLITS * SM_TOTAL + EM_SPLITS * EM_TOTAL;
 }
 
-extern "C" int toued_lpg_wgrad(const int32_t* obs, const uint8_t* done, const float* critic,
-                               const float* lpg_params, const float* x, const float* h, const float* dgates,
-                               const float* d_pi_hat, const float* dl, const float* dx, float* workspace,
-                               int n_agents, int n_workers, int rollout_len, int obs_dim,
+extern "C" int toued_lpg_wgrad(const float* tok_y, const uint8_t* done, const float* lpg_params, const float* x,
+                               const float* h, const float* dgates, const float* d_pi_hat, const float* dl,
+                               const float* dx, float* workspace, int n_agents, int n_workers, int rollout_len,
                                int lifetime_conditioning, int accumulate, void* stream) {
     const int R = n_agents * n_workers, L = rollout_len;
     TOUED_CHECK(R > 0 && L > 0, "toued_lpg_wgrad: empty problem");
@@ -459,8 +455,8 @@
         TOUED_LAUNCH_CHECK();
     }
     TOUED_CUDA(cudaFuncSetAttribute(embed_backward_kernel, cudaFuncAttributeMaxDynamicSharedMemorySize, EM_SMEM));
-    embed_backward_kernel<<<EM_SPLITS, 256, EM_SMEM, st>>>(obs, done, critic, lpg_params, lpg_offsets(lifetime_conditioning ? 7 : 5).e_w0,
-                                                      dx, p_em, nullptr, n_agents, n_workers, L, obs_dim, accumulate);
+    embed_backward_kernel<<<EM_SPLITS, 256, EM_SMEM, st>>>(tok_y, done, lpg_params, lpg_offsets(lifetime_conditioning ? 7 : 5).e_w0,
+                                                      dx, p_em, nullptr, n_agents, n_workers, L, accumulate);
     TOUED_LAUNCH_CHECK();
     return 0;
 }
@@ -507,15 +503,14 @@
     return WG_SPLITS * LPG_H * LPG_G + SM_SPLITS * SM_TOTAL;
 }
 
-extern "C" int toued_lpg_wgrad_embed(const int32_t* obs, const uint8_t* done, const float* critic, const float* lpg_params,
-                                     const float* dx, float* workspace, const uint32_t* cotangent_max, int n_agents,
-                                     int n_workers, int rollout_len, int obs_dim, int lifetime_conditioning, int accumulate,
-                                     void* stream) {
+extern "C" int toued_lpg_wgrad_embed(const float* tok_y, const uint8_t* done, const float* lpg_params, const float* dx,
+                                     float* workspace, const uint32_t* cotangent_max, int n_agents, int n_workers,
+                                     int rollout_len, int lifetime_conditioning, int accumulate, void* stream) {
     float* p_em = workspace + toued_lpg_wgrad_workspace_offset(2);
     TOUED_CUDA(cudaFuncSetAttribute(embed_backward_kernel, cudaFuncAttributeMaxDynamicSharedMemorySize, EM_SMEM));
     embed_backward_kernel<<<EM_SPLITS, 256, EM_SMEM, (cudaStream_t)stream>>>(
-        obs, done, critic, lpg_params, lpg_offsets(lifetime_conditioning ? 7 : 5).e_w0, dx, p_em, cotangent_max, n_agents,
-        n_workers, rollout_len, obs_dim, accumulate);
+        tok_y, done, lpg_params, lpg_offsets(lifetime_conditioning ? 7 : 5).e_w0, dx, p_em, cotangent_max, n_agents,
+        n_workers, rollout_len, accumulate);
     TOUED_LAUNCH_CHECK();
     return 0;
 }
diff --git a/to_ued_b200/csrc/lpg_common.cuh b/to_ued_b200/csrc/lpg_common.cuh
--- a/to_ued_b200/csrc/lpg_common.cuh
+++ b/to_ued_b200/csrc/lpg_common.cuh
@@ -67,6 +67,27 @@
     for (int j = 0; j < C; ++j) z[j] = r[j] + tf * l[j];
 }
 
+__device__ __forceinline__ void load_row8(const float* __restrict__ src, float (&v)[8]) {
+    const float4 a = reinterpret_cast<const float4*>(src)[0], b = reinterpret_cast<const float4*>(src)[1];
+    v[0] = a.x; v[1] = a.y; v[2] = a.z; v[3] = a.w; v[4] = b.x; v[5] = b.y; v[6] = b.z; v[7] = b.w;
+}
+template <int C>
+__device__ __forceinline__ void load_row8(const float* __restrict__ src, float (&v)[C]) {
+    float r[8];
+    load_row8(src, r);
+#pragma unroll
+    for (int j = 0; j < C; ++j) v[j] = r[j];
+}
+template <int C>
+__device__ __forceinline__ void store_row8(float* __restrict__ dst, const float (&v)[C]) {
+    float r[8];
+#pragma unroll
+    for (int j = 0; j < 8; ++j) r[j] = j < C ? v[j] : 0.0f;
+    float4* o = reinterpret_cast<float4*>(dst);
+    o[0] = make_float4(r[0], r[1], r[2], r[3]);
+    o[1] = make_float4(r[4], r[5], r[6], r[7]);
+}
+
 __device__ __forceinline__ float block_sum(float v, float* red) {
 #pragma unroll
     for (int o = 16; o > 0; o >>= 1) v += __shfl_xor_sync(0xffffffffu, v, o);
diff --git a/to_ued_b200/csrc/lpg_forward.cu b/to_ued_b200/csrc/lpg_forward.cu
--- a/to_ued_b200/csrc/lpg_forward.cu
+++ b/to_ued_b200/csrc/lpg_forward.cu
@@ -130,6 +130,7 @@
                    const float* __restrict__ actor, const float* __restrict__ critic,
                    const float* __restrict__ lpg, const int32_t* __restrict__ step,
                    const LevelRec* __restrict__ levels, float* __restrict__ x, unsigned char* __restrict__ ximg,
+                   float* __restrict__ tok_p, float* __restrict__ tok_y,
                    int n_agents, int W, int L, int D, int cond, int emb_off, int lpg_stride) {
     __shared__ float sp_s[LPG_Y * LPG_E + LPG_E + LPG_E + 1];
     if (lpg_stride == 0) {
@@ -159,6 +160,12 @@
     softmax_c<LPG_Y>(zy, y0);
     tab_logits8<LPG_Y>(ct, D, ob1, zy);
     softmax_c<LPG_Y>(zy, y1);
+    if (tok_p) {
+        const size_t yi = ((size_t)n * (L + 1) + t) * W + w;
+        store_row8(tok_p + g * 8, p);
+        store_row8(tok_y + yi * 8, y0);
+        if (t == L - 1) store_row8(tok_y + (yi + W) * 8, y1);
+    }
     const float d = done[g] ? 1.0f : 0.0f;
     float pyt, pyt1;
     embed_mlp2(y0, y1, sp, pyt, pyt1);
@@ -179,19 +186,31 @@
     }
 }
 
+extern "C" int toued_lpg_prepare_rec(const int32_t* obs, const uint8_t* action, const float* reward,
+                                     const uint8_t* done, const float* actor, const float* critic,
+                                     const float* lpg_params, const int32_t* step, const void* levels,
+                                     float* x, void* ximg, float* tok_p, float* tok_y, int n_agents, int n_workers,
+                                     int rollout_len, int obs_dim, int lifetime_conditioning, int lpg_stride,
+                                     void* stream) {
+    const size_t total = (size_t)n_agents * rollout_len * n_workers;
+    TOUED_CHECK(total > 0, "toued_lpg_prepare: empty problem");
+    TOUED_CHECK((tok_p == nullptr) == (tok_y == nullptr), "toued_lpg_prepare_rec: tok_p and tok_y go together");
+    lpg_prepare_kernel<<<(unsigned)((total + 255) / 256), 256, 0, (cudaStream_t)stream>>>(
+        obs, action, reward, done, actor, critic, lpg_params, step, (const LevelRec*)levels, x, (unsigned char*)ximg,
+        tok_p, tok_y, n_agents, n_workers, rollout_len, obs_dim, lifetime_conditioning,
+        lpg_offsets(lifetime_conditioning ? 7 : 5).e_w0, lpg_stride);
+    TOUED_LAUNCH_CHECK();
+    return 0;
+}
+
 extern "C" int toued_lpg_prepare(const int32_t* obs, const uint8_t* action, const float* reward,
                                  const uint8_t* done, const float* actor, const float* critic,
                                  const float* lpg_params, const int32_t* step, const void* levels,
                                  float* x, void* ximg, int n_agents, int n_workers, int rollout_len, int obs_dim,
                                  int lifetime_conditioning, int lpg_stride, void* stream) {
-    const size_t total = (size_t)n_agents * rollout_len * n_workers;
-    TOUED_CHECK(total > 0, "toued_lpg_prepare: empty problem");
-    lpg_prepare_kernel<<<(unsigned)((total + 255) / 256), 256, 0, (cudaStream_t)stream>>>(
-        obs, action, reward, done, actor, critic, lpg_params, step, (const LevelRec*)levels, x, (unsigned char*)ximg,
-        n_agents, n_workers, rollout_len, obs_dim, lifetime_conditioning,
-        lpg_offsets(lifetime_conditioning ? 7 : 5).e_w0, lpg_stride);
-    TOUED_LAUNCH_CHECK();
-    return 0;
+    return toued_lpg_prepare_rec(obs, action, reward, done, actor, critic, lpg_params, step, levels, x, ximg, nullptr,
+                                 nullptr, n_agents, n_workers, rollout_len, obs_dim, lifetime_conditioning, lpg_stride,
+                                 stream);
 }
 
 constexpr int GF_TM = 64;
diff --git a/to_ued_b200/meta/train.py b/to_ued_b200/meta/train.py
--- a/to_ued_b200/meta/train.py
+++ b/to_ued_b200/meta/train.py
@@ -236,8 +236,8 @@
 
     def _agent_backward(ws, tape, k, buf, s):
         _lib.call("toued_agent_backward", p(tape.obs[k]), p(tape.action[k]), p(tape.sorted_tok[k]),
-                  p(tape.pi_hat[k]), p(tape.y_hat[k]), p(tape.actor[k]), p(tape.critic[k]),
-                  p(tape.actor[k + 1]), p(tape.critic[k + 1]), p(tape.scalars[k]), p(ws.lam), p(ws.mu),
+                  p(tape.pi_hat[k]), p(tape.y_hat[k]), p(tape.tok_p[k]), p(tape.tok_y[k]),
+                  p(tape.tok_p1[k]), p(tape.tok_y1[k]), p(tape.scalars[k]), p(ws.lam), p(ws.mu),
                   p(ws.d_pi_hat2[buf]), p(ws.d_y_hat2[buf]), nb, W, L, D, float(actor.learning_rate),
                   float(critic.learning_rate), float(actor.max_grad_norm),
                   float(lpg_hypers.agent_target_coeff), *[float(b) for b in bK], float(gscale), p(ws.ab_scratch), s)
@@ -252,9 +252,9 @@
                 _agent_backward(ws, tape, k, 0, s)
                 _lib.call("toued_gru_backward", p(tape.done[k]), p(lpg), p(ws.whT), p(tape.h[k]), p(tape.gates[k]),
                           p(tape.y_hat[k]), p(ws.d_pi_hat), p(ws.d_y_hat), p(ws.dl), p(ws.dx), nb, W, L, cond, s)
-                _lib.call("toued_lpg_wgrad", p(tape.obs[k]), p(tape.done[k]), p(tape.critic[k]), p(lpg), p(tape.x[k]),
+                _lib.call("toued_lpg_wgrad", p(tape.tok_y[k]), p(tape.done[k]), p(lpg), p(tape.x[k]),
                           p(tape.h[k]), p(tape.gates[k]), p(ws.d_pi_hat), p(ws.dl), p(ws.dx), p(ws.partials),
-                          nb, W, L, D, cond, 0 if first else 1, s)
+                          nb, W, L, cond, 0 if first else 1, s)
             return
         ev, buf = evs[mb], k & 1
         for d in ("ab", "bwd", "wg", "em"):
@@ -292,8 +292,8 @@
         with torch.cuda.stream(em_streams[slot]):
             st = em_streams[slot]
             st.wait_event(ev["bwd"][k])
-            _lib.call("toued_lpg_wgrad_embed", p(tape.obs[k]), p(tape.done[k]), p(tape.critic[k]), p(lpg),
-                      p(ws.dx2[buf]), p(ws.partials), p(ws.cotmax[k:k + 1]), nb, W, L, D, cond, 0 if first else 1,
+            _lib.call("toued_lpg_wgrad_embed", p(tape.tok_y[k]), p(tape.done[k]), p(lpg),
+                      p(ws.dx2[buf]), p(ws.partials), p(ws.cotmax[k:k + 1]), nb, W, L, cond, 0 if first else 1,
                       _lib.stream_ptr())
             ev["em"][k].record(st)
 
```
